# suilin0432/SoS-WSOD

Hardware: AMD Instinct MI355X
Metric: images/s (1/2/4/8 MI355X) VGG16+OICR 2000-prop; conv5_3 MFMA-util % (higher is better)
Workload: dtype bf16; 1 GPU; OICR+ training iteration: 4 views/step/GPU (1 image(s) x 2 scales x h-flip, every view 512x512), R=2000 proposals/view, K=20, VGG16 dilated-C5 + ROIPool 7x7 + fc6/fc7 4096 + WSDDN + 4 OICR heads, fwd+bwd+SGD(momentum, wd); image=one view, parallelism=dp1

## Files before the change

### include/soswsod_hip.h

```cpp
#ifndef SOSWSOD_HIP_H
#define SOSWSOD_HIP_H

#include <stdint.h>

#ifdef __cplusplus
extern "C" {
#endif

#ifndef SW_F32
#define SW_F32 0
#define SW_BF16 1
#endif

typedef struct ihipStream_t* sw_stream_t;

typedef struct sw_epilogue {
  const float* bias;
  int relu;
  const uint8_t* drop_mask;
  long ld_drop;
  float drop_scale;
  const void* relu_ref;
  long ld_ref;
  float ref_scale;
  int ref_dtype;
  int out_dtype;
  int accumulate_atomic;
  float* absmax_out;
  uint64_t drop_seed, drop_offset;
  float drop_hash_p;
  const uint64_t* drop_offset_dev;
  float* splitk_workspace;
  const void* residual;
  long ld_res;
  int res_dtype;
  const float* fold_row_scale;
  const struct sw_sgd_tensor_s* sgd_fused;
  float sgd_momentum, sgd_grad_scale;
} sw_epilogue;

int sw_gemm(int dtype, int a_kstrided, int b_kstrided, int M, int N, int K, const void* A, long lda, const void* B,
            long ldb, void* C, long ldc, const sw_epilogue* ep, int splitk, sw_stream_t stream);
long sw_gemm_splitk_workspace_floats(int M, int N, int K, int splitk);

int sw_conv3x3_igemm(int dtype, int nimg, int H, int W, int Cin, int Cout, int dilation, const void* in,
                     const void* wk, void* out, const sw_epilogue* ep, sw_stream_t stream);
int sw_conv3x3_relu_pool2(int dtype, int nimg, int H, int W, int Cin, int Cout, const void* in, const void* wk, const float* bias,
                          void* out_pooled, sw_stream_t stream);
typedef struct sw_conv_problem {
  int32_t nimg, H, W, Cin, Cout;
  const void* in; const void* wk; void* out;
  const sw_epilogue* ep;
} sw_conv_problem;
int sw_conv3x3_multi(int dtype, int n, const sw_conv_problem* probs, sw_stream_t stream);
long sw_conv3x3_wgrad_workspace_floats(int dtype, int nimg, int H, int W, int Cin, int Cout, int splitk);
int sw_conv3x3_wgrad(int dtype, int nimg, int H, int W, int Cin, int Cout, int dilation, const void* x, const void* dy,
                     float* dw_oihw, float* workspace, int splitk, const float* cout_scale, int accumulate, sw_stream_t stream);
int sw_conv3x3_wgrad_small(int dtype, int nimg, int H, int W, int Cin, int Cout, const void* x, const void* dy,
                           const float* cout_scale, float* dw_oihw, int accumulate, sw_stream_t stream);
int sw_conv3x3_wgrad_fold(int Cin, int Cout, int nslab, const float* workspace, float* dw_oihw, const float* cout_scale,
                          int accumulate, sw_stream_t stream);
typedef struct {
  int nimg, H, W, Cin, Cout, dilation, nsplit;
  const void* x;
  const void* dy;
  float* slabs;
} sw_wgrad_problem;
int sw_conv3x3_wgrad_grouped(int dtype, int n_problems, const sw_wgrad_problem* problems, sw_stream_t stream);
typedef struct sw_gemm_kk_problem {
  const void* A; const void* B; float* slabs;
  int32_t M, N, K, nsplit;
  long lda, ldb;
} sw_gemm_kk_problem;
int sw_gemm_kk_grouped(int dtype, int n_problems, const sw_gemm_kk_problem* problems, sw_stream_t stream);
long sw_gemm_kk_grouped_slabs(int dtype, int K, int nsplit);
typedef struct sw_splitk_fold { int32_t M, N, nslab, accumulate; const float* workspace; float* C; long ldc; const float* row_scale; } sw_splitk_fold;
int sw_splitk_fold_multi(int n, const sw_splitk_fold* folds, sw_stream_t stream);
typedef struct { int Cin, Cout, nslab; const float* workspace; float* dw_oihw; } sw_wgrad_fold;
int sw_conv3x3_wgrad_fold_multi(int n, const sw_wgrad_fold* folds, sw_stream_t stream);
int sw_conv_weight_prep(int dtype, int mode, int Cout, int Cin, int cin_pad, const float* w_oihw, void* wk,
                        sw_stream_t stream);

int sw_maxpool2x2_fwd(int dtype, int nimg, int H, int W, int C, int stride, const void* in, void* out,
                      sw_stream_t stream);
int sw_maxpool2x2_bwd(int dtype, int nimg, int H, int W, int C, int stride, const void* in, const void* dout,
                      void* din, int relu_mask, sw_stream_t stream);

int sw_preprocess(int dtype, int H, int W, int cpad, const uint8_t* img_chw, const float* mean3,
                  const float* std3, void* out_nhwc, sw_stream_t stream);
int sw_preprocess_multi(int dtype, int n, int H, int W, int cpad, const uint8_t* const* imgs_chw, const float* mean3,
                        const float* std3, void* out_nhwc, sw_stream_t stream);

long sw_roi_pool_fwd_workspace_bytes(int nimg, int R, int PH, int PW);
int sw_roi_pool_fwd(int dtype, int nimg, int H, int W, int C, int PH, int PW, float spatial_scale, const void* feat,
                    const float* rois, int R, const float* row_scale, float row_scale_add, void* out,
                    void* argmax, int argmax_bits, long ld_out, void* workspace, long workspace_bytes, sw_stream_t stream);
int sw_roi_pool_bwd(int dtype, int nimg, int H, int W, int C, int PH, int PW, const void* dout,
                    const void* argmax, int argmax_bits, long ld_in, const float* rois, int R, const float* row_scale,
                    float row_scale_add, const void* relu_ref, const float* dout_absmax, void* dfeat, float spatial_scale,
                    sw_stream_t stream);
int sw_absmax(int dtype, long n, const void* x, float* out, sw_stream_t stream);

long sw_wsddn_workspace_floats(int V, int R, int K);
int sw_wsddn_mil(int V, int R, int K, const float* logits, long ld, int cls_col, int det_col, const float* gt_onehot,
                 float* scores, float* loss_view, float* dlogits, long ld_d, const float* grad_scale,
                 float* mean_scores, long ld_mean, float* workspace, sw_stream_t stream);

long sw_wsddn_scores_bwd_workspace_floats(int R, int K);
int sw_wsddn_scores_bwd(int R, int K, const float* logits, long ld, const float* g_scores, long ld_g, float* dlogits, long ld_d,
                        float* workspace, sw_stream_t stream);
int sw_mean_views(int V, long n, const float* in, float* out, sw_stream_t stream);

int sw_oicr_mean_probs(int V, int R, int K, int n_rounds, const float* logits, long ld, int cls_col0, int col_stride,
                       float* out, sw_stream_t stream);

long sw_mine_workspace_bytes(int R, int top_k, int G);
int sw_oicr_mine_label(int R, int ncol, int K, int n_rounds, const float* scores, const int32_t* gt_classes, int G,
                       const float* boxes, int top_k, float score_thresh, float nms_thresh, float iou_bg,
                       float iou_fg, int32_t* lab_class, float* lab_weight, int32_t* lab_index, int32_t* pgt_count,
                       int32_t* pgt_index, int32_t* pgt_class, float* pgt_score, void* workspace,
                       sw_stream_t stream);

int sw_oicr_refine_loss(int V, int R, int K, int n_rounds, const float* logits, long ld, int cls_col, int box_col,
                        int col_stride, const float* boxes, const int32_t* lab_class, const float* lab_weight,
                        const int32_t* lab_index, const int32_t* pred_view, const float* reg_weights4,
                        float* loss_view, float* dlogits, long ld_d, const float* grad_scale, float* workspace,
                        sw_stream_t stream);

int sw_focal_loss(int N, int C, const float* logits, long ld, const int32_t* targets, float gamma, float* loss,
// ... 211 lines not shown
```

### sos-wsod_amd/_lib.py

```python
import ctypes
import os

import torch

_HERE = os.path.dirname(os.path.abspath(__file__))
LIB_PATH = os.environ.get("SW_LIB_PATH") or os.path.join(_HERE, "libsoswsod_hip.so")

SW_F32, SW_BF16 = 0, 1

c_int, c_long, c_float, c_void_p, c_u64 = ctypes.c_int, ctypes.c_long, ctypes.c_float, ctypes.c_void_p, ctypes.c_uint64
c_int32, c_uint32, c_double, c_longlong = ctypes.c_int32, ctypes.c_uint32, ctypes.c_double, ctypes.c_longlong


class Epilogue(ctypes.Structure):
    _fields_ = [
        ("bias", c_void_p), ("relu", c_int), ("drop_mask", c_void_p), ("ld_drop", c_long), ("drop_scale", c_float),
        ("relu_ref", c_void_p), ("ld_ref", c_long), ("ref_scale", c_float), ("ref_dtype", c_int),
        ("out_dtype", c_int), ("accumulate_atomic", c_int), ("absmax_out", c_void_p),
        ("drop_seed", c_u64), ("drop_offset", c_u64), ("drop_hash_p", c_float), ("drop_offset_dev", c_void_p),
        ("splitk_workspace", c_void_p),
        ("residual", c_void_p), ("ld_res", c_long), ("res_dtype", c_int),
        ("fold_row_scale", c_void_p),
        ("sgd_fused", c_void_p), ("sgd_momentum", c_float), ("sgd_grad_scale", c_float),
    ]


class WgradProblem(ctypes.Structure):
    _fields_ = [("nimg", c_int), ("H", c_int), ("W", c_int), ("Cin", c_int), ("Cout", c_int),
                ("dilation", c_int), ("nsplit", c_int), ("x", c_void_p), ("dy", c_void_p),
                ("slabs", c_void_p)]


class WgradFold(ctypes.Structure):
    _fields_ = [("Cin", c_int), ("Cout", c_int), ("nslab", c_int), ("workspace", c_void_p),
                ("dw_oihw", c_void_p)]


class AugRecipe(ctypes.Structure):
    _fields_ = [("seed", c_u64), ("key", c_u64), ("order", c_int32 * 4), ("factor", c_float * 4),
                ("hue_shift", c_int32), ("grayscale", c_int32), ("blur_r", c_int32),
                ("blur_ww", c_uint32), ("blur_fw", c_uint32), ("rect", (c_int32 * 4) * 3),
                ("pad_", c_int32)]


class AugItem(ctypes.Structure):
    _fields_ = [("src", c_void_p), ("out", c_void_p), ("tmp", c_void_p), ("lsum", c_void_p),
                ("H", c_int32), ("W", c_int32), ("recipe", AugRecipe)]


class GemmKKProblem(ctypes.Structure):
    _fields_ = [("A", c_void_p), ("B", c_void_p), ("slabs", c_void_p), ("M", c_int32), ("N", c_int32),
                ("K", c_int32), ("nsplit", c_int32), ("lda", c_long), ("ldb", c_long)]


class SplitkFold(ctypes.Structure):
    _fields_ = [("M", c_int32), ("N", c_int32), ("nslab", c_int32), ("accumulate", c_int32),
                ("workspace", c_void_p), ("C", c_void_p), ("ldc", c_long), ("row_scale", c_void_p)]


class ConvProblem(ctypes.Structure):
    _fields_ = [("nimg", c_int32), ("H", c_int32), ("W", c_int32), ("Cin", c_int32), ("Cout", c_int32),
                ("in_", c_void_p), ("wk", c_void_p), ("out", c_void_p), ("ep", ctypes.POINTER(Epilogue))]


class CopyDesc(ctypes.Structure):
    _fields_ = [("src", c_void_p), ("dst", c_void_p), ("bytes", c_long)]


class ColsumPart(ctypes.Structure):
    _fields_ = [("M", c_int), ("N", c_int), ("X", c_void_p), ("ld", c_long), ("workspace", c_void_p)]


class StageDesc(ctypes.Structure):
    _fields_ = [("w", c_void_p), ("bn_weight", c_void_p), ("bn_bias", c_void_p), ("bn_mean", c_void_p), ("bn_var", c_void_p),
                ("scale", c_void_p), ("shift", c_void_p), ("dst", c_void_p),
                ("kind", c_int32), ("rows", c_int32), ("cols", c_int32), ("block_start", c_int32)]


class ColsumFold(ctypes.Structure):
    _fields_ = [("N", c_int), ("n_partial_rows", c_int), ("workspace", c_void_p), ("out", c_void_p)]


class SgdTensor(ctypes.Structure):
    _fields_ = [
        ("param", c_void_p), ("grad", c_void_p), ("momentum_buf", c_void_p), ("n", c_long), ("lr", c_float),
        ("weight_decay", c_float), ("first_step", c_int), ("stage_kind", c_int), ("stage_dtype", c_int),
        ("stage0", c_void_p), ("stage1", c_void_p), ("d0", c_int), ("d1", c_int), ("d2", c_int), ("ld0", c_long), ("ld1", c_long),
        ("hyper_dev", c_void_p),
    ]


SGD_MAX_TENSORS = 24
_EP = ctypes.POINTER(Epilogue)
_F4 = ctypes.POINTER(c_float)

SIGNATURES = {
    "sw_gemm": (c_int, [c_int, c_int, c_int, c_int, c_int, c_int, c_void_p, c_long, c_void_p, c_long, c_void_p, c_long,
                        _EP, c_int, c_void_p]),
    "sw_gemm_splitk_workspace_floats": (c_long, [c_int, c_int, c_int, c_int]),
    "sw_gemm_sgd_fused_supported": (c_int, [c_int, c_int, c_int, c_int, c_int, c_int]),
    "sw_conv3x3_igemm": (c_int, [c_int, c_int, c_int, c_int, c_int, c_int, c_int, c_void_p, c_void_p, c_void_p, _EP,
                                 c_void_p]),
    "sw_conv3x3_wgrad": (c_int, [c_int, c_int, c_int, c_int, c_int, c_int, c_int, c_void_p, c_void_p, c_void_p, c_void_p,
                                 c_int, c_void_p, c_int, c_void_p]),
    "sw_conv3x3_wgrad_workspace_floats": (c_long, [c_int, c_int, c_int, c_int, c_int, c_int, c_int]),
    "sw_conv_weight_prep": (c_int, [c_int, c_int, c_int, c_int, c_int, c_void_p, c_void_p, c_void_p]),
    "sw_maxpool2x2_fwd": (c_int, [c_int, c_int, c_int, c_int, c_int, c_int, c_void_p, c_void_p, c_void_p]),
    "sw_maxpool2x2_bwd": (c_int, [c_int, c_int, c_int, c_int, c_int, c_int, c_void_p, c_void_p, c_void_p, c_int,
                                  c_void_p]),
    "sw_preprocess": (c_int, [c_int, c_int, c_int, c_int, c_void_p, _F4, _F4, c_void_p, c_void_p]),
    "sw_preprocess_multi": (c_int, [c_int, c_int, c_int, c_int, c_int, ctypes.POINTER(c_void_p), _F4, _F4, c_void_p, c_void_p]),
    "sw_roi_pool_fwd": (c_int, [c_int, c_int, c_int, c_int, c_int, c_int, c_int, c_float, c_void_p, c_void_p, c_int,
                                c_void_p, c_float, c_void_p, c_void_p, c_int, c_long, c_void_p, c_long, c_void_p]),
    "sw_roi_pool_fwd_workspace_bytes": (c_long, [c_int, c_int, c_int, c_int]),
    "sw_roi_pool_bwd": (c_int, [c_int, c_int, c_int, c_int, c_int, c_int, c_int, c_void_p, c_void_p, c_int, c_long, c_void_p, c_int,
                                c_void_p, c_float, c_void_p, c_void_p, c_void_p, c_float, c_void_p]),
    "sw_absmax": (c_int, [c_int, c_long, c_void_p, c_void_p, c_void_p]),
    "sw_wsddn_workspace_floats": (c_long, [c_int, c_int, c_int]),
    "sw_wsddn_mil": (c_int, [c_int, c_int, c_int, c_void_p, c_long, c_int, c_int, c_void_p, c_void_p, c_void_p,
                             c_void_p, c_long, c_void_p, c_void_p, c_long, c_void_p, c_void_p]),
    "sw_mean_views": (c_int, [c_int, c_long, c_void_p, c_void_p, c_void_p]),
    "sw_oicr_mean_probs": (c_int, [c_int, c_int, c_int, c_int, c_void_p, c_long, c_int, c_int, c_void_p, c_void_p]),
    "sw_mine_workspace_bytes": (c_long, [c_int, c_int, c_int]),
    "sw_oicr_mine_label": (c_int, [c_int, c_int, c_int, c_int, c_void_p, c_void_p, c_int, c_void_p, c_int, c_float, c_float,
                                   c_float, c_float, c_void_p, c_void_p, c_void_p, c_void_p, c_void_p, c_void_p,
                                   c_void_p, c_void_p, c_void_p]),
    "sw_oicr_refine_loss": (c_int, [c_int, c_int, c_int, c_int, c_void_p, c_long, c_int, c_int, c_int, c_void_p, c_void_p,
                                    c_void_p, c_void_p, c_void_p, _F4, c_void_p, c_void_p, c_long, c_void_p,
                                    c_void_p, c_void_p]),
    "sw_oicr_predict": (c_int, [c_int, c_int, c_int, c_void_p, c_long, c_int, c_int, c_void_p, _F4, c_float, c_void_p,
                                c_void_p, c_void_p]),
    "sw_detect_workspace_bytes": (c_long, [c_int, c_int, c_int]),
    "sw_detect_postprocess": (c_int, [c_int, c_int, c_void_p, c_void_p, c_int, c_int, c_float, c_float, c_int, c_void_p,
                                      c_void_p, c_void_p, c_void_p, c_void_p, c_void_p, c_long, c_void_p]),
    "sw_tta_merge": (c_int, [c_int, c_int, c_int, c_void_p, c_void_p, c_void_p, c_void_p, c_void_p, c_int, c_int, c_float, c_int,
                             c_void_p, c_void_p, c_void_p, c_void_p, c_void_p, c_void_p]),
    "sw_colsum": (c_int, [c_int, c_int, c_int, c_void_p, c_long, c_void_p, c_void_p, c_int, c_void_p]),
    "sw_colsum_workspace_floats": (c_long, [c_int, c_int, c_int]),
    "sw_conv3x3_wgrad_small": (c_int, [c_int, c_int, c_int, c_int, c_int, c_int, c_void_p, c_void_p, c_void_p, c_void_p, c_int, c_void_p]),
    "sw_conv3x3_wgrad_fold": (c_int, [c_int, c_int, c_int, c_void_p, c_void_p, c_void_p, c_int, c_void_p]),
    "sw_conv3x3_wgrad_fold_multi": (c_int, [c_int, ctypes.POINTER(WgradFold), c_void_p]),
    "sw_conv3x3_multi": (c_int, [c_int, c_int, ctypes.POINTER(ConvProblem), c_void_p]),
    "sw_gemm_kk_grouped": (c_int, [c_int, c_int, ctypes.POINTER(GemmKKProblem), c_void_p]),
    "sw_gemm_kk_grouped_slabs": (c_long, [c_int, c_int, c_int]),
    "sw_splitk_fold_multi": (c_int, [c_int, ctypes.POINTER(SplitkFold), c_void_p]),
    "sw_colsum_fold_multi": (c_int, [c_int, ctypes.POINTER(ColsumFold), c_void_p]),
    "sw_colsum_partial_multi": (c_int, [c_int, c_int, ctypes.POINTER(ColsumPart), c_void_p]),
    "sw_conv3x3_wgrad_grouped": (c_int, [c_int, c_int, ctypes.POINTER(WgradProblem), c_void_p]),
    "sw_convert_2d": (c_int, [c_int, c_int, c_int, c_void_p, c_long, c_void_p, c_long, c_void_p]),
    "sw_split_bf16x3": (c_int, [c_int, c_int, c_void_p, c_long, c_void_p, c_long, c_int, c_int, c_void_p]),
    "sw_nchw_to_nhwc": (c_int, [c_int, c_int, c_int, c_int, c_int, c_int, c_void_p, c_void_p, c_void_p]),
    "sw_relu_bwd": (c_int, [c_int, c_long, c_void_p, c_void_p, c_void_p, c_void_p]),
    "sw_scale_cols": (c_int, [c_int, c_int, c_int, c_void_p, c_long, c_void_p, c_void_p, c_long, c_void_p]),
    "sw_fill_zero": (c_int, [c_void_p, c_long, c_void_p]),
    "sw_dropout_mask": (c_int, [c_void_p, c_long, c_u64, c_u64, c_float, c_void_p]),
    "sw_sgd_momentum_step": (c_int, [c_void_p, c_void_p, c_void_p, c_long, c_float, c_float, c_float, c_int, c_float,
                                     c_void_p]),
    "sw_convert_2d_t": (c_int, [c_int, c_int, c_int, c_void_p, c_long, c_void_p, c_long, c_void_p]),
    "sw_sgd_multi": (c_int, [c_int, ctypes.POINTER(SgdTensor), c_float, c_float, c_void_p]),
    "sw_loss_finalize": (c_int, [c_int, c_int, c_int, c_void_p, c_void_p, c_void_p, c_void_p]),
    "sw_scale_cols_loss": (c_int, [c_int, c_int, c_int, c_int, c_void_p, c_long, c_void_p, c_void_p, c_void_p, c_float,
                                   c_void_p, c_long, c_void_p]),
    "sw_resize_pass_u8": (c_int, [c_int, c_int, c_int, c_long, c_long, c_int, c_int, c_void_p, c_void_p, c_void_p, c_int, c_void_p,
                                  c_void_p, c_void_p]),
    "sw_color_jitter_u8": (c_int, [c_int, c_int, c_int, c_void_p, c_float, c_double, c_float, c_void_p, c_void_p, c_void_p]),
    "sw_transpose_2d": (c_int, [c_int, c_int, c_int, c_void_p, c_long, c_void_p, c_long, c_void_p]),
    "sw_stage_blocks": (c_int, [c_int, c_int, c_int]),
    "sw_stage_weights_multi": (c_int, [c_int, c_int, c_void_p, c_int, c_float, c_void_p]),
    "sw_ema_multi": (c_int, [c_int, ctypes.POINTER(c_void_p), ctypes.POINTER(c_void_p), ctypes.POINTER(c_long), c_double, c_void_p]),
    "sw_threshold_select": (c_int, [c_int, c_void_p, c_void_p, c_void_p, c_float, c_void_p, c_int, c_void_p, c_void_p, c_void_p,
                                    c_void_p, c_void_p, c_void_p]),
    "sw_conv3x3_relu_pool2": (c_int, [c_int, c_int, c_int, c_int, c_int, c_int, c_void_p, c_void_p, c_void_p, c_void_p, c_void_p]),
    "sw_weighted_sum": (c_int, [c_int, c_void_p, c_void_p, c_void_p, c_void_p]),
    "sw_scale_scalars": (c_int, [c_int, c_void_p, c_void_p, c_void_p, c_void_p]),
    "sw_counter_add": (c_int, [c_void_p, c_u64, c_void_p]),
    "sw_focal_loss": (c_int, [c_int, c_int, c_void_p, c_long, c_void_p, c_float, c_void_p, c_void_p, c_long, c_void_p, c_void_p]),
    "sw_gaussian_blur_weights": (c_int, [c_float, ctypes.POINTER(c_int32), ctypes.POINTER(c_uint32),
                                         ctypes.POINTER(c_uint32)]),
    "sw_strong_aug_workspace_bytes": (c_long, [c_int, c_int]),
    "sw_strong_aug_u8": (c_int, [c_int, c_int, c_void_p, ctypes.POINTER(AugRecipe), c_void_p, c_void_p, c_void_p]),
    "sw_strong_aug_multi_u8": (c_int, [c_int, c_void_p, c_int, c_int, c_int, c_void_p]),
    "sw_copy_multi": (c_int, [c_int, ctypes.POINTER(CopyDesc), c_void_p]),
    "sw_pack_views": (c_int, [c_int, ctypes.POINTER(c_void_p), ctypes.POINTER(c_void_p), c_void_p, c_void_p, c_void_p,
                              c_void_p]),
    "sw_preprocess_pad": (c_int, [c_int, c_int, c_int, c_int, c_int, c_void_p, _F4, _F4, c_void_p, c_void_p]),
# ... 77 lines not shown
```

### sos-wsod_amd/backbone_vgg.py

```python
import os

import torch
import torch.nn as nn

from . import ops, staging
from .registry import BACKBONE_REGISTRY
from .structures import ShapeSpec

_STAGES = [("plain1", 3, 64, 2), ("plain2", 64, 128, 2), ("plain3", 128, 256, 3), ("plain4", 256, 512, 3),
           ("plain5", 512, 512, 3)]


def _epc(dtype):
    return 8 if dtype == torch.bfloat16 else 4


class _Conv(nn.Module):

    def __init__(self, cin, cout):
        super().__init__()
        self.weight = nn.Parameter(torch.empty(cout, cin, 3, 3))
        self.bias = nn.Parameter(torch.zeros(cout))
        nn.init.kaiming_normal_(self.weight, mode="fan_out", nonlinearity="relu")

# ... 134 lines not shown
                pi += 2
                cin = cur.shape[3]
                if (ci == blk.num_conv - 1 and blk.has_pool and blk.pool_stride == 2 and blk.dilation == 1 and dtype == torch.bfloat16
                        and (ft is None or bi < ft[0]) and cur.shape[1] >= 2 and cur.shape[2] >= 2):
                    oh, ow = (cur.shape[1] - 2) // 2 + 1, (cur.shape[2] - 2) // 2 + 1
                    pooled = torch.empty(cur.shape[0], oh, ow, blk.out_channels, device=x.device, dtype=dtype)
                    if ops.conv3x3_relu_pool2(cur, module.staged_weight(w, 0, cin, dtype), b, pooled, tag=f"{blk.tag}.conv{ci + 1}_fwd"):
                        conv_io.append((cur, None))
                        cur = pooled
                        continue
                out = torch.empty(cur.shape[0], cur.shape[1], cur.shape[2], blk.out_channels, device=x.device, dtype=dtype)
                ep = ops.make_epilogue(bias=b, relu=True, out_dtype=dtype)
                if module.x3_layer(dtype, cin, blk.out_channels):
                    n_, h_, w_ = cur.shape[:3]
                    x3 = ops.split_bf16x3(cur.view(n_ * h_ * w_, cin), 0,
                                          out=torch.empty(n_ * h_ * w_, 6 * cin, device=x.device, dtype=torch.bfloat16))
                    ops.conv3x3(x3.view(n_, h_, w_, 6 * cin), module.staged_weight_x3(w, 0, cin), out, blk.dilation, ep,
                                tag=f"{blk.tag}.conv{ci + 1}_fwd")
                else:
                    wk = module.staged_weight(w, 0, cin, dtype)
                    ops.conv3x3(cur, wk, out, blk.dilation, ep, tag=f"{blk.tag}.conv{ci + 1}_fwd")
                conv_io.append((cur, out))
                cur = out
            pre_pool = None
            if blk.has_pool and conv_io[-1][1] is not None:
                pre_pool = cur
                s = blk.pool_stride
                oh, ow = (cur.shape[1] - 2) // s + 1, (cur.shape[2] - 2) // s + 1
                pooled = torch.empty(cur.shape[0], oh, ow, cur.shape[3], device=x.device, dtype=dtype)
                ops.maxpool_fwd(cur, pooled, s)
                cur = pooled
            stage_info.append((conv_io, pre_pool))
        return cur, stage_info

    @staticmethod
    def backward(ctx, *gs):
        module, infos, params = ctx.module, ctx.infos, ctx.params
        ctx.infos = None
        n_in = len(infos)
        grads = [None] * len(params)
        first_trainable = module.first_trainable_conv()
        live = [i for i in range(n_in) if gs[i] is not None]
        if first_trainable is None or not live:
            return (None, None) + (None,) * n_in + tuple(grads)
        dev = gs[live[0]].device
        dtype = infos[0][0][0][0][0].dtype
        main = torch.cuda.current_stream()
        side = module.side_stream() if len(live) > 1 else None
        x3w = False
        if module.fp32x3 and dtype == torch.float32:
            x3w, pj = True, len(params)
            for sj in range(len(module.blocks) - 1, -1, -1):
                for cj in range(module.blocks[sj].num_conv - 1, -1, -1):
                    pj -= 2
                    if params[pj].requires_grad and not module.x3_layer(dtype, infos[live[0]][sj][0][cj][0].shape[3], module.blocks[sj].out_channels):
                        x3w = False
        wdt, nmul = (torch.bfloat16, 6) if x3w else (dtype, 1)
        bk = 64 if wdt == torch.bfloat16 else 32
        deferred = []
        module._colsum_deferred = []
        shapes, probs6, keys = [], [], []
        pj = len(params)
        for sj in range(len(module.blocks) - 1, -1, -1):
            bj = module.blocks[sj]
            for cj in range(bj.num_conv - 1, -1, -1):
                pj -= 2
                if params[pj].requires_grad:
                    for i in live:
                        xin = infos[i][sj][0][cj][0]
                        shapes.append((nmul * xin.shape[0] * xin.shape[1] * xin.shape[2], bj.out_channels, 9 * xin.shape[3]))
                        probs6.append((nmul * xin.shape[0], xin.shape[1], xin.shape[2], xin.shape[3], bj.out_channels, bj.dilation))
                        keys.append((pj, i))
        direct_ns = dict(zip(keys, _wgrad_direct_splits(probs6))) if _wgrad_direct_covers(probs6, wdt) else None
        target = _wgrad_grouped_target(shapes, bk)
        plan = {}
        pidx = len(params)
        for si in range(len(module.blocks) - 1, -1, -1):
            blk = module.blocks[si]
            for ci in range(blk.num_conv - 1, -1, -1):
                pidx -= 2
                w = params[pidx]
                if w.requires_grad:
                    cout = blk.out_channels
                    slab_off, row_off, nslab, nrow, splits = {}, {}, 0, 0, {}
                    for i in live:
                        x_in = infos[i][si][0][ci][0]
                        n, H, W, cin = x_in.shape
                        splits[i] = (direct_ns[(pidx, i)] if direct_ns is not None
                                     else _wgrad_grouped_splits(nmul * n * H * W, bk, target))
                        slab_off[i], row_off[i] = nslab, nrow
                        nslab += ops.conv3x3_wgrad_nslab_shape(wdt, nmul * n, H, W, cin, cout, splits[i])
                        nrow += ops.colsum_nrows(dtype, n * H * W, cout)
                    cin = infos[live[0]][si][0][ci][0].shape[3]
                    plan[pidx] = dict(ws=torch.empty(nslab, cout * 9 * cin, device=dev, dtype=torch.float32),
                                      rows=torch.empty(nrow, cout, device=dev, dtype=torch.float32), slab_off=slab_off,
                                      row_off=row_off, nslab=nslab, nrow=nrow, splits=splits, cin=cin,
                                      dw=ops.grad_target(w, (cout, cin, 3, 3), dev),
                                      db=ops.grad_target(params[pidx + 1], (cout,), dev))
                if (si, ci) == first_trainable:
                    break
            if si == first_trainable[0]:
                break
        if side is not None:
            side.wait_stream(main)
        for k, i in enumerate(live):
            st = side if (side is not None and k % 2 == 1) else main
            with torch.cuda.stream(st):
                g = gs[i]
                if st is not main:
                    g.record_stream(st)
                _VGGFunction._backward_one(module, infos[i], params, g, dtype, plan, i, first_trainable,
                                           deferred, None if st is main else main, x3w)
            infos[i] = None
        if side is not None:
            main.wait_stream(side)
        if deferred:
            ops.conv3x3_wgrad_grouped(deferred, tag="wgrad_grouped")
            ops.colsum_partial_multi(module._colsum_deferred)
            deferred.clear()
        module._colsum_deferred = []
        ops.conv3x3_wgrad_fold_multi([(pl["ws"], pl["nslab"], pl["dw"]) for pl in plan.values()])
        ops.colsum_fold_multi([(pl["rows"], pl["nrow"], pl["db"]) for pl in plan.values()])
        for pidx, pl in plan.items():
            w = params[pidx]
            grads[pidx] = pl["dw"][:, : w.shape[1]].contiguous() if pl["cin"] != w.shape[1] else pl["dw"]
            grads[pidx + 1] = pl["db"]
        return (None, None) + (None,) * n_in + tuple(grads)

    @staticmethod
    def _backward_one(module, stage_info, params, g, dtype, plan, i, first_trainable, deferred, consumer_stream, x3w=False):
        g = g.contiguous()
        if g.dtype != dtype:
            g = g.to(dtype)
        last_out = stage_info[-1][0][-1][1]
        assert stage_info[-1][1] is None, "backward expects the last stage to have no pool (vgg.py:197)"
        dz = ops.relu_bwd(last_out, g, out=torch.empty_like(g))
        pidx = len(params)
        for si in range(len(stage_info) - 1, -1, -1):
            blk = module.blocks[si]
            conv_io, _ = stage_info[si]
            for ci in range(blk.num_conv - 1, -1, -1):
                pidx -= 2
                x_in, _ = conv_io[ci]
                w = params[pidx]
                n, H, W, cin = x_in.shape
                pl = plan.get(pidx)
                if pl is not None:
                    npix = n * H * W
                    xw, dw_ = x_in, dz
                    if x3w:
                        cout = blk.out_channels
                        xw = ops.split_bf16x3(x_in.view(npix, cin), 1, along_rows=True,
                                              out=torch.empty(6 * npix, cin, device=g.device, dtype=torch.bfloat16)).view(6 * n, H, W, cin)
                        dw_ = ops.split_bf16x3(dz.view(npix, cout), 0, along_rows=True,
                                               out=torch.empty(6 * npix, cout, device=g.device, dtype=torch.bfloat16)).view(6 * n, H, W, cout)
                    if consumer_stream is not None:
                        xw.record_stream(consumer_stream); dw_.record_stream(consumer_stream)
                        dz.record_stream(consumer_stream)
                    deferred.append((xw, dw_, pl["ws"][pl["slab_off"][i]:], blk.dilation, pl["splits"][i]))
                    module._colsum_deferred.append((dz.view(npix, blk.out_channels), pl["rows"][pl["row_off"][i]:]))
                if (si, ci) == first_trainable:
                    return
                dx = torch.empty(n, H, W, cin, device=g.device, dtype=dtype)
                ref = x_in.view(n * H * W, cin) if ci > 0 else None
                epd = ops.make_epilogue(relu_ref=ref, out_dtype=dtype)
                if module.x3_layer(dtype, blk.out_channels, cin):
                    cout = blk.out_channels
                    dz3 = ops.split_bf16x3(dz.view(n * H * W, cout), 0,
                                           out=torch.empty(n * H * W, 6 * cout, device=g.device, dtype=torch.bfloat16))
                    ops.conv3x3(dz3.view(n, H, W, 6 * cout), module.staged_weight_x3(w, 1, cin), dx, blk.dilation, epd,
                                tag=f"{blk.tag}.conv{ci + 1}_dgrad")
                else:
                    wkd = module.staged_weight(w, 1, cin, dtype)
                    ops.conv3x3(dz, wkd, dx, blk.dilation, epd, tag=f"{blk.tag}.conv{ci + 1}_dgrad")
                dz = dx
            prev_pre_pool = stage_info[si - 1][1]
            pblk = module.blocks[si - 1]
            din = torch.empty_like(prev_pre_pool)
            ops.maxpool_bwd(prev_pre_pool, dz, din, pblk.pool_stride, relu_mask=True)
            dz = din


class VGG16(nn.Module):

    def __init__(self, conv5_dilation, freeze_at, num_classes=None, out_features=None, compute_dtype=torch.bfloat16):
        super().__init__()
        self.num_classes = num_classes
        self.compute_dtype = compute_dtype
        self.dual_stream = True
        self._side = None
        self._stage = staging.StageCache()
        self._stage_x3 = staging.StageCache()
        self.fp32x3 = (compute_dtype == torch.float32 and os.environ.get("SW_FP32X3", "0") == "1"
                       and os.environ.get("SW_FP32X3_CONV", "1") != "0")
        self._out_feature_strides, self._out_feature_channels = {}, {}
        self.stages_and_names = []
        strides = {"plain1": 2, "plain2": 4, "plain3": 8, "plain4": 8 if conv5_dilation == 2 else 16,
                   "plain5": 8 if conv5_dilation == 2 else 16}
        self.blocks = []
        for i, (name, cin, cout, nconv) in enumerate(_STAGES):
            if name == "plain4":
                blk = PlainBlock(cin, cout, num_conv=nconv, stride=1 if conv5_dilation == 2 else 2, has_pool=True)
            elif name == "plain5":
                blk = PlainBlock(cin, cout, num_conv=nconv, stride=1, dilation=conv5_dilation, has_pool=False)
            else:
                blk = PlainBlock(cin, cout, num_conv=nconv, stride=2, has_pool=True)
            stage = nn.Sequential(blk)
            self.add_module(name, stage)
            self.stages_and_names.append((stage, name))
            blk.tag = name
            self.blocks.append(blk)
            self._out_feature_strides[name] = strides[name]
            self._out_feature_channels[name] = cout
            if freeze_at >= i + 1:
                blk.freeze()
        if out_features is None:
            out_features = ["plain5"]
        self._out_features = out_features
        assert self._out_features == ["plain5"], "this build exposes the hot path's feature only (IN_FEATURES ['plain5'])"

    @property
    def size_divisibility(self):
        return 0

    def staged_weight(self, w, mode, cin_pad, dtype):
        cout, cin = w.shape[:2]
        shape = (cout, 9, cin_pad) if mode == 0 else (cin, 9, cout)
        slot, built = self._stage.lookup((id(w), mode), (w,), (shape,), dtype, w.device, alloc=torch.zeros,
                                         build=lambda b: ops.conv_weight_prep(w.detach(), b[0], mode, cin_pad if mode == 0 else None))
        if built and w.requires_grad:
            both = [self._stage.get((id(w), m)) for m in (0, 1)]
            both = [s if s is not None and s.bufs[0].dtype == dtype else None for s in both]
            b0, b1 = (None if s is None else s.bufs[0] for s in both)
            staging.register(w, 2, dtype, stage0=b0, stage1=b1, d0=cout, d1=cin, d2=cin if b0 is None else b0.shape[2],
                             slots=[(s, 0) for s in both if s is not None])
        return slot.bufs[0]

    def x3_layer(self, dtype, cin, cout):
        return self.fp32x3 and dtype == torch.float32 and cin % 64 == 0 and cout % 64 == 0

    def staged_weight_x3(self, w, mode, cin_pad):
        n, k = (w.shape[0], cin_pad) if mode == 0 else (w.shape[1], w.shape[0])
        return self._stage_x3.lookup((id(w), mode), (w,), ((n, 9, 6 * k),), torch.bfloat16, w.device, lambda b: ops.split_bf16x3(
            self.staged_weight(w, mode, cin_pad, torch.float32).view(9 * n, k), 1, out=b[0].view(9 * n, 6 * k)))[0].bufs[0]

    def stage_all_weights(self, with_dgrad):
        dtype = self.compute_dtype
        epc = _epc(dtype)
# ... 67 lines not shown
```

### sos-wsod_amd/csrc/conv_direct.hip

```cpp
#include <type_traits>
#include "common.h"
#include "soswsod_hip.h"

namespace {

constexpr int TH = 8, TW = 32, CK = 32;
constexpr unsigned INVALID = 0xFFFFFF00u;

struct DirectArgs {
  const void* in; const void* wk; void* out;
  const float* bias; const void* ref;
  int nimg, H, W, Cin, Cout, relu;
  int pool;
  int out_f32;
  int tiles_x, tiles_y, n_px_tiles, n_co_blocks, total;
  unsigned in_bytes, wk_bytes;
};

template <int N> __device__ __forceinline__ void wait_vm() { asm volatile("s_waitcnt vmcnt(%0)" ::"n"(N) : "memory"); }

template <int DIL, int TN, int KG = 1>
__device__ __forceinline__ void conv3x3_direct_body(const DirectArgs& g, const unsigned bid) {
  static_assert(KG == 1 || (KG == 2 && TN == 64), "K groups: two groups of four waves, 64-channel tiles");
  constexpr int DEPTH = 2;
  constexpr int NI = TN / 16;
  constexpr int B_INSTR = 3 * TN * 4 / 64, B_PER_WAVE = (B_INSTR + 3) / 4;
  constexpr int PH = TH + 2 * DIL, PW = TW + 2 * DIL, P = PH * PW;
  constexpr int A_INSTR = (P * 4 + 63) / 64;
  constexpr int A_PER_WAVE = (A_INSTR + 3) / 4;
  constexpr int A_BYTES = A_PER_WAVE * 4 * 1024;
  constexpr int B_BYTES = 3 * TN * 64;
  typedef __attribute__((address_space(3))) void* lvoid;
  extern __shared__ __attribute__((aligned(16))) char smem[];
  const int tid = threadIdx.x, lane = tid & 63;
  const int wave_all = __builtin_amdgcn_readfirstlane(tid >> 6);
  const int grp = KG == 1 ? 0 : (wave_all >> 2), wave = wave_all & 3;
  char* const sA = smem + grp * (2 * A_BYTES);
  char* const sB = smem + KG * 2 * A_BYTES + grp * (DEPTH * B_BYTES);

  const int per_xcd = (g.total + 7) >> 3;
  const int f = (bid & 7) * per_xcd + (bid >> 3);
  if ((int)(bid >> 3) >= per_xcd || f >= g.total) return;
  const int px_tile = f / g.n_co_blocks, co_blk = f - px_tile * g.n_co_blocks;
  const int img = px_tile / (g.tiles_x * g.tiles_y);
  const int trem = px_tile - img * (g.tiles_x * g.tiles_y);
  const int ty0 = (trem / g.tiles_x) * TH, tx0 = (trem % g.tiles_x) * TW;
  const int co0 = co_blk * TN;

  const __amdgpu_buffer_rsrc_t rsA = __builtin_amdgcn_make_buffer_rsrc((void*)g.in, 0, (int)g.in_bytes, 0x00020000);
  const __amdgpu_buffer_rsrc_t rsB = __builtin_amdgcn_make_buffer_rsrc((void*)g.wk, 0, (int)g.wk_bytes, 0x00020000);

  unsigned a_v[A_PER_WAVE];
#pragma unroll
  for (int s = 0; s < A_PER_WAVE; ++s) {
    const int q = wave + 4 * s;
    const int idx = q * 64 + lane;
    const int prow = idx >> 2, p = idx & 3;
    const int src = p ^ (((prow >> 2) & 1) << 1);
    const int py = prow / PW, px = prow - py * PW;
    const int y = ty0 - DIL + py, x = tx0 - DIL + px;
    const bool ok = prow < P && y >= 0 && y < g.H && x >= 0 && x < g.W;
    a_v[s] = ok ? (unsigned)(((((long)img * g.H + y) * g.W + x) * g.Cin + src * 8) * 2) : INVALID;
  }
  unsigned b_v[B_PER_WAVE];
#pragma unroll
  for (int s = 0; s < B_PER_WAVE; ++s) {
    const int idx = (wave + 4 * s) * 64 + lane;
    const int r = idx >> 2, p = idx & 3;
    const int tap_x = r / TN, co = r - tap_x * TN;
    const int src = p ^ (((co >> 2) & 1) << 1);
    const bool ok = tap_x < 3 && co0 + co < g.Cout;
    b_v[s] = ok ? (unsigned)((((long)(co0 + co) * 9 + tap_x) * g.Cin + src * 8) * 2) : INVALID;
  }
  auto issue_a = [&](int chunk) {
    char* dst = sA + (chunk & 1) * A_BYTES;
    const unsigned soff = (unsigned)(chunk * KG + grp) * (CK * 2);
#pragma unroll
    for (int s = 0; s < A_PER_WAVE; ++s)
      __builtin_amdgcn_raw_ptr_buffer_load_lds(rsA, (lvoid)(dst + (wave + 4 * s) * 1024), 16, (int)a_v[s], (int)soff, 0, 0);
  };
  auto issue_b = [&](int step) {
    const int chunk = step / 3, ty = step - chunk * 3;
    char* dst = sB + (step % DEPTH) * B_BYTES;
    const unsigned soff = (unsigned)((ty * 3 * g.Cin + (chunk * KG + grp) * CK) * 2);
#pragma unroll
    for (int s = 0; s < B_PER_WAVE; ++s)
      if (wave + 4 * s < B_INSTR)
        __builtin_amdgcn_raw_ptr_buffer_load_lds(rsB, (lvoid)(dst + (wave + 4 * s) * 1024), 16, (int)b_v[s], (int)soff, 0, 0);
  };

  f32x4 acc[4][NI];
#pragma unroll
  for (int i = 0; i < 4; ++i)
#pragma unroll
    for (int j = 0; j < NI; ++j) acc[i][j] = f32x4{0.f, 0.f, 0.f, 0.f};

  const int nchunk = g.Cin / (CK * KG), nstep = nchunk * 3;
  const int l15 = lane & 15, kq = lane >> 4;
  int b_off[NI];
#pragma unroll
// ... 48 lines not shown
        if (step + 1 < nstep) issue_b(step + 1);
        if (ty == 0 && chunk + 1 < nchunk) issue_a(chunk + 1);
        if (FORM != FORM_EMPTY) compute_step(par_c, ty_c);
      };
      one(std::integral_constant<int, 0>{}); one(std::integral_constant<int, 1>{}); one(std::integral_constant<int, 2>{});
    };
    for (int chunk = 0; chunk < nchunk; chunk += 2) {
      chunk_steps(std::integral_constant<int, 0>{}, chunk);
      if (chunk + 1 < nchunk) chunk_steps(std::integral_constant<int, 1>{}, chunk + 1);
    }
  };
  {
    static_assert(TW == 32 && TH == 8, "edge forms: 16-pixel sub-tiles, two rows per wave");
    const bool left_only = tx0 + 16 >= g.W;
    const bool no_rows = ty0 + 2 * wave >= g.H;
    if (no_rows) main_loop(std::integral_constant<int, FORM_EMPTY>{});
    else if (left_only) main_loop(std::integral_constant<int, FORM_LEFT>{});
    else main_loop(std::integral_constant<int, FORM_FULL>{});
  }
  __syncthreads();

  unsigned short* out = (unsigned short*)g.out;
  const unsigned short* ref = (const unsigned short*)g.ref;
  if (KG == 2) {
    f32x4* X = (f32x4*)smem;
#pragma unroll
    for (int i2 = 0; i2 < 2; ++i2)
#pragma unroll
      for (int j = 0; j < NI; ++j) {
        const f32x4 give = grp == 0 ? acc[2 + i2][j] : acc[i2][j];
        X[((wave_all * 2 + i2) * NI + j) * 64 + lane] = give;
      }
    __syncthreads();
    f32x4 fin[2][NI];
#pragma unroll
    for (int i2 = 0; i2 < 2; ++i2)
#pragma unroll
      for (int j = 0; j < NI; ++j) {
        const f32x4 got = X[(((wave_all ^ 4) * 2 + i2) * NI + j) * 64 + lane];
        const f32x4 mine = grp == 0 ? acc[i2][j] : acc[2 + i2][j];
        fin[i2][j] = grp == 0 ? f32x4{mine[0] + got[0], mine[1] + got[1], mine[2] + got[2], mine[3] + got[3]}
                              : f32x4{got[0] + mine[0], got[1] + mine[1], got[2] + mine[2], got[3] + mine[3]};
      }
    if (g.out_f32) {
      float* outf = (float*)g.out;
      const float* reff = (const float*)g.ref;
      const int y = ty0 + 2 * wave + grp;
#pragma unroll
      for (int j = 0; j < NI; ++j) {
        const int co = co0 + j * 16 + l15;
        const float bv = (g.bias && co < g.Cout) ? g.bias[co] : 0.f;
#pragma unroll
        for (int i2 = 0; i2 < 2; ++i2)
#pragma unroll
          for (int e = 0; e < 4; ++e) {
            const int x = tx0 + i2 * 16 + kq * 4 + e;
            if (y < g.H && x < g.W && co < g.Cout) {
              float v = fin[i2][j][e] + bv;
              if (g.relu) v = relu_keep_nan(v);
              const long o = (((long)img * g.H + y) * g.W + x) * g.Cout + co;
              if (reff && !(reff[o] > 0.f)) v = 0.f;
              outf[o] = v;
            }
          }
      }
      return;
    }
    unsigned short* S = (unsigned short*)(smem + 8 * 2 * NI * 64 * 16 + wave_all * (32 * TN * 2));
#pragma unroll
    for (int j = 0; j < NI; ++j) {
      const int col = j * 16 + l15;
      const float bv = (g.bias && co0 + col < g.Cout) ? g.bias[co0 + col] : 0.f;
#pragma unroll
      for (int i2 = 0; i2 < 2; ++i2)
#pragma unroll
        for (int e = 0; e < 4; ++e) {
          float v = fin[i2][j][e] + bv;
          if (g.relu) v = relu_keep_nan(v);
          const int pl = i2 * 16 + kq * 4 + e;
          S[pl * TN + (col ^ ((pl & (TN / 8 - 1)) << 3))] = f32_to_bf16_bits(v);
        }
    }
    __builtin_amdgcn_s_waitcnt(0xc07f);
#pragma unroll
    for (int it = 0; it < TN / 16; ++it) {
      const int idx = it * 64 + lane;
      const int pl = idx / (TN / 8), ch = idx % (TN / 8);
      const int y = ty0 + 2 * wave + grp, x = tx0 + pl;
      const int co = co0 + ch * 8;
      if (y < g.H && x < g.W && co < g.Cout) {
        u32x4 v = *(const u32x4*)(S + pl * TN + ((ch ^ (pl & (TN / 8 - 1))) << 3));
        const long o = (((long)img * g.H + y) * g.W + x) * g.Cout + co;
        if (ref) {
          const u32x4 r = *(const u32x4*)(ref + o);
#pragma unroll
          for (int t = 0; t < 4; ++t) {
            const bool lo = __uint_as_float(r[t] << 16) > 0.f, hi = __uint_as_float(r[t] & 0xFFFF0000u) > 0.f;
            v[t] = (lo ? (v[t] & 0xFFFFu) : 0u) | (hi ? (v[t] & 0xFFFF0000u) : 0u);
          }
        }
        *(u32x4*)(out + o) = v;
      }
    }
    return;
  }
  if (g.out_f32) {
    float* outf = (float*)g.out;
    const float* reff = (const float*)g.ref;
#pragma unroll
    for (int j = 0; j < NI; ++j) {
      const int co = co0 + j * 16 + l15;
      const float bv = (g.bias && co < g.Cout) ? g.bias[co] : 0.f;
#pragma unroll
      for (int i = 0; i < 4; ++i)
#pragma unroll
        for (int e = 0; e < 4; ++e) {
          const int pl = i * 16 + kq * 4 + e;
          const int y = ty0 + 2 * wave + (pl >> 5), x = tx0 + (pl & 31);
          if (y < g.H && x < g.W && co < g.Cout) {
            float v = acc[i][j][e] + bv;
            if (g.relu) v = relu_keep_nan(v);
            const long o = (((long)img * g.H + y) * g.W + x) * g.Cout + co;
            if (reff && !(reff[o] > 0.f)) v = 0.f;
            outf[o] = v;
          }
        }
    }
    return;
  }
  unsigned short* S = (unsigned short*)(smem + wave * (64 * TN * 2));
#pragma unroll
  for (int j = 0; j < NI; ++j) {
    const int col = j * 16 + l15;
    const float bv = (g.bias && co0 + col < g.Cout) ? g.bias[co0 + col] : 0.f;
#pragma unroll
    for (int i = 0; i < 4; ++i)
#pragma unroll
      for (int e = 0; e < 4; ++e) {
        float v = acc[i][j][e] + bv;
        if (g.relu) v = relu_keep_nan(v);
        const int pl = i * 16 + kq * 4 + e;
        S[pl * TN + (col ^ ((pl & (TN / 8 - 1)) << 3))] = f32_to_bf16_bits(v);
      }
  }
  __builtin_amdgcn_s_waitcnt(0xc07f);
  if (g.pool) {
    const int OH = (g.H - 2) / 2 + 1, OW = (g.W - 2) / 2 + 1;
#pragma unroll
    for (int it = 0; it < (16 * (TN / 8) + 63) / 64; ++it) {
      const int idx = it * 64 + lane;
      const int pp = idx / (TN / 8), ch = idx % (TN / 8);
      const int oy = (ty0 + 2 * wave) >> 1, ox = (tx0 >> 1) + pp;
      const int co = co0 + ch * 8;
      if (pp < 16 && oy < OH && ox < OW && co < g.Cout) {
        float a[8];
#pragma unroll
        for (int t = 0; t < 4; ++t) {
          const int pl = (t >> 1) * 32 + 2 * pp + (t & 1);
          const u32x4 v = *(const u32x4*)(S + pl * TN + ((ch ^ (pl & (TN / 8 - 1))) << 3));
#pragma unroll
          for (int q = 0; q < 4; ++q) {
            const float lo = __uint_as_float(v[q] << 16), hi = __uint_as_float(v[q] & 0xFFFF0000u);
            a[2 * q] = t == 0 ? lo : max_keep_nan(a[2 * q], lo);
            a[2 * q + 1] = t == 0 ? hi : max_keep_nan(a[2 * q + 1], hi);
          }
        }
        u32x4 o;
#pragma unroll
        for (int q = 0; q < 4; ++q) o[q] = (unsigned)f32_to_bf16_bits(a[2 * q]) | ((unsigned)f32_to_bf16_bits(a[2 * q + 1]) << 16);
        *(u32x4*)(out + (((long)img * OH + oy) * OW + ox) * g.Cout + co) = o;
      }
    }
    return;
  }
#pragma unroll
  for (int it = 0; it < TN / 8; ++it) {
    const int idx = it * 64 + lane;
    const int pl = idx / (TN / 8), ch = idx % (TN / 8);
    const int y = ty0 + 2 * wave + (pl >> 5), x = tx0 + (pl & 31);
    const int co = co0 + ch * 8;
    if (y < g.H && x < g.W && co < g.Cout) {
      u32x4 v = *(const u32x4*)(S + pl * TN + ((ch ^ (pl & (TN / 8 - 1))) << 3));
      const long o = (((long)img * g.H + y) * g.W + x) * g.Cout + co;
      if (ref) {
        const u32x4 r = *(const u32x4*)(ref + o);
#pragma unroll
        for (int t = 0; t < 4; ++t) {
          const bool lo = __uint_as_float(r[t] << 16) > 0.f, hi = __uint_as_float(r[t] & 0xFFFF0000u) > 0.f;
          v[t] = (lo ? (v[t] & 0xFFFFu) : 0u) | (hi ? (v[t] & 0xFFFF0000u) : 0u);
        }
      }
      *(u32x4*)(out + o) = v;
    }
  }
}

template <int DIL, int TN, int KG = 1>
__global__ __launch_bounds__(256 * KG, KG == 1 ? 2 : 1) void conv3x3_direct_kernel(DirectArgs g) {
  conv3x3_direct_body<DIL, TN, KG>(g, blockIdx.x);
}

constexpr int DIRECT_MULTI_MAX = 8;
struct DirectMulti {
  int n;
  unsigned first[DIRECT_MULTI_MAX + 1];
  DirectArgs p[DIRECT_MULTI_MAX];
};
__global__ __launch_bounds__(256, 2) void conv3x3_direct_multi_kernel(DirectMulti m) {
  int i = 0;
  while (i + 1 < m.n && blockIdx.x >= m.first[i + 1]) ++i;
  conv3x3_direct_body<1, 64, 1>(m.p[i], blockIdx.x - m.first[i]);
}

__global__ __launch_bounds__(256) void conv3x3_first_kernel(int nimg, int H, int W, const unsigned short* __restrict__ in,
                                                            const unsigned short* __restrict__ wk,
                                                            const float* __restrict__ bias, int relu,
                                                            unsigned short* __restrict__ out) {
  __shared__ __attribute__((aligned(16))) unsigned short S_all[4][64 * 64];
  const int lane = threadIdx.x & 63, wave = threadIdx.x >> 6;
  const int l15 = lane & 15, kq = lane >> 4;
  unsigned short* S = S_all[wave];
  u32x4 fb[4][3];
#pragma unroll
  for (int j = 0; j < 4; ++j)
#pragma unroll
    for (int s3 = 0; s3 < 3; ++s3) {
      const int tap = s3 * 4 + kq;
      fb[j][s3] = tap < 9 ? *(const u32x4*)(wk + ((long)(j * 16 + l15) * 9 + tap) * 8) : u32x4{0u, 0u, 0u, 0u};
    }
  float bv[4];
#pragma unroll
  for (int j = 0; j < 4; ++j) bv[j] = bias ? bias[j * 16 + l15] : 0.f;
  int dy[3], dx[3];
#pragma unroll
  for (int s3 = 0; s3 < 3; ++s3) { const int tap = s3 * 4 + kq; dy[s3] = tap / 3 - 1; dx[s3] = tap % 3 - 1; }
  const int segs = (W + 63) / 64;
  const long nseg = (long)nimg * H * segs;
  for (long sg = (long)blockIdx.x * 4 + wave; sg < nseg; sg += (long)gridDim.x * 4) {
    const int xs = (int)(sg % segs) * 64; const long t = sg / segs;
    const int y = (int)(t % H), img = (int)(t / H);
    f32x4 acc[4][4];
#pragma unroll
    for (int i = 0; i < 4; ++i)
#pragma unroll
      for (int j = 0; j < 4; ++j) acc[i][j] = f32x4{0.f, 0.f, 0.f, 0.f};
#pragma unroll
    for (int i = 0; i < 4; ++i) {
      const int x = xs + i * 16 + l15;
      u32x4 fa[3];
#pragma unroll
      for (int s3 = 0; s3 < 3; ++s3) {
        const int yy = y + dy[s3], xx = x + dx[s3];
        const bool ok = s3 * 4 + kq < 9 && yy >= 0 && yy < H && xx >= 0 && xx < W;
        fa[s3] = ok ? *(const u32x4*)(in + (((long)img * H + yy) * W + xx) * 8) : u32x4{0u, 0u, 0u, 0u};
      }
#pragma unroll
      for (int s3 = 0; s3 < 3; ++s3)
#pragma unroll
        for (int j = 0; j < 4; ++j)
          acc[i][j] = __builtin_amdgcn_mfma_f32_16x16x32_bf16(__builtin_bit_cast(bf16x8, fa[s3]), __builtin_bit_cast(bf16x8, fb[j][s3]),
                                                              acc[i][j], 0, 0, 0);
    }
#pragma unroll
    for (int j = 0; j < 4; ++j)
#pragma unroll
      for (int i = 0; i < 4; ++i)
#pragma unroll
        for (int e = 0; e < 4; ++e) {
          float v = acc[i][j][e] + bv[j];
          if (relu) v = relu_keep_nan(v);
          const int pl = i * 16 + kq * 4 + e, col = j * 16 + l15;
          S[pl * 64 + (col ^ ((pl & 7) << 3))] = f32_to_bf16_bits(v);
        }
#pragma unroll
    for (int it = 0; it < 8; ++it) {
      const int idx = it * 64 + lane;
      const int pl = idx >> 3, ch = idx & 7;
      const int x = xs + pl;
      if (x < W)
        *(u32x4*)(out + (((long)img * H + y) * W + x) * 64 + ch * 8) = *(const u32x4*)(S + pl * 64 + ((ch ^ (pl & 7)) << 3));
    }
  }
}

}

int sw_conv3x3_direct_try(int nimg, int H, int W, int Cin, int Cout, int dilation, const void* in, const void* wk, void* out,
                          const sw_epilogue* ep, hipStream_t stream) {
  if (Cin == 8 && Cout == 64 && dilation == 1 && ep && ep->out_dtype == SW_BF16 && !ep->drop_mask && !ep->relu_ref &&
      !ep->accumulate_atomic && !ep->absmax_out && !(ep->drop_hash_p > 0.f) &&
      (((uintptr_t)in | (uintptr_t)wk | (uintptr_t)out) & 15) == 0) {
    const long nseg = (long)nimg * H * ((W + 63) / 64);
    long blocks = (nseg + 3) / 4;
    if (blocks > 4096) blocks = 4096;
    hipLaunchKernelGGL(conv3x3_first_kernel, dim3((unsigned)blocks), dim3(256), 0, stream, nimg, H, W, (const unsigned short*)in,
                       (const unsigned short*)wk, ep->bias, ep->relu, (unsigned short*)out);
    hipError_t e1 = hipGetLastError();
    return e1 == hipSuccess ? 1 : -(int)e1;
  }
  if ((Cin % CK) || (Cout % 8) || (dilation != 1 && dilation != 2)) return 0;
  if (ep && ((ep->out_dtype != SW_BF16 && ep->out_dtype != SW_F32) || ep->drop_mask || ep->accumulate_atomic || ep->absmax_out)) return 0;
  if (!ep) return 0;
  if (ep->relu_ref && (ep->ref_dtype != ep->out_dtype || ep->ld_ref != Cout || ep->ref_scale != 1.0f)) return 0;
  if (ep->residual || ep->drop_hash_p > 0.f) return 0;
  if ((((uintptr_t)in | (uintptr_t)wk | (uintptr_t)out | (uintptr_t)ep->relu_ref) & 15)) return 0;
  if (Cin < 64) return 0;
  DirectArgs g = {};
  g.in = in; g.wk = wk; g.out = out; g.bias = ep->bias; g.ref = ep->relu_ref; g.relu = ep->relu;
  g.out_f32 = ep->out_dtype == SW_F32;
  g.nimg = nimg; g.H = H; g.W = W; g.Cin = Cin; g.Cout = Cout;
  g.tiles_x = (W + TW - 1) / TW; g.tiles_y = (H + TH - 1) / TH;
  g.n_px_tiles = g.tiles_x * g.tiles_y * nimg;
  const bool few = g.n_px_tiles * ((Cout + 63) / 64) <= 384;
  const int kg = (few && (Cin % (2 * CK)) == 0) ? 2 : 1;
  const int tn = (few && kg == 1) ? 32 : 64;
  g.n_co_blocks = (Cout + tn - 1) / tn;
  g.total = g.n_px_tiles * g.n_co_blocks;
  const long ib = (long)nimg * H * W * Cin * 2, wb = (long)Cout * 9 * Cin * 2;
  if (ib >= 0xFFFFFF00L || wb >= 0xFFFFFF00L) return 0;
  g.in_bytes = (unsigned)ib; g.wk_bytes = (unsigned)wb;
  const int per_xcd = (g.total + 7) / 8;
  const int d = dilation;
  const int P = (TH + 2 * d) * (TW + 2 * d);
  const int apw = ((P * 4 + 63) / 64 + 3) / 4;
  const size_t lds = (size_t)kg * ((size_t)2 * apw * 4096 + (size_t)2 * (3 * tn * 64));
  hipError_t e = hipSuccess;
#define SW_LAUNCH_DIRECT(D, TNV, KGV)                                                                                     \
  do {                                                                                                                     \
    auto kern = conv3x3_direct_kernel<D, TNV, KGV>;                                                                        \
    e = hipFuncSetAttribute((const void*)kern, hipFuncAttributeMaxDynamicSharedMemorySize, (int)lds);                      \
    if (e != hipSuccess) return -(int)e;                                                                                   \
    hipLaunchKernelGGL(kern, dim3(per_xcd * 8), dim3(256 * kg), lds, stream, g);                                           \
  } while (0)
  if (kg == 2) { if (d == 1) SW_LAUNCH_DIRECT(1, 64, 2); else SW_LAUNCH_DIRECT(2, 64, 2); }
  else if (tn == 32) { if (d == 1) SW_LAUNCH_DIRECT(1, 32, 1); else SW_LAUNCH_DIRECT(2, 32, 1); }
  else { if (d == 1) SW_LAUNCH_DIRECT(1, 64, 1); else SW_LAUNCH_DIRECT(2, 64, 1); }
#undef SW_LAUNCH_DIRECT
  e = hipGetLastError();
  if (e != hipSuccess) return -(int)e;
  return 1;
}


extern "C" int sw_conv3x3_relu_pool2(int dtype, int nimg, int H, int W, int Cin, int Cout, const void* in, const void* wk, const float* bias,
                                     void* out_pooled, hipStream_t stream) {
  SW_ENTER();
  if (dtype != SW_BF16 || (Cin % CK) || Cin < 64 || (Cout % 64) || H < 2 || W < 2) return 0;
  if ((((uintptr_t)in | (uintptr_t)wk | (uintptr_t)out_pooled) & 15)) return 0;
  DirectArgs g = {};
  g.in = in; g.wk = wk; g.out = out_pooled; g.bias = bias; g.ref = nullptr; g.relu = 1; g.pool = 1;
  g.nimg = nimg; g.H = H; g.W = W; g.Cin = Cin; g.Cout = Cout;
  g.tiles_x = (W + TW - 1) / TW; g.tiles_y = (H + TH - 1) / TH;
  g.n_px_tiles = g.tiles_x * g.tiles_y * nimg;
  g.n_co_blocks = Cout / 64;
  g.total = g.n_px_tiles * g.n_co_blocks;
  if (g.total <= 384) return 0;
  const long ib = (long)nimg * H * W * Cin * 2, wb = (long)Cout * 9 * Cin * 2;
  if (ib >= 0xFFFFFF00L || wb >= 0xFFFFFF00L) return 0;
  g.in_bytes = (unsigned)ib; g.wk_bytes = (unsigned)wb;
  const int per_xcd = (g.total + 7) / 8;
  constexpr int P = (TH + 2) * (TW + 2);
  constexpr int apw = ((P * 4 + 63) / 64 + 3) / 4;
  const size_t lds = (size_t)2 * apw * 4096 + (size_t)2 * (3 * 64 * 64);
  auto kern = conv3x3_direct_kernel<1, 64, 1>;
  hipError_t e = hipFuncSetAttribute((const void*)kern, hipFuncAttributeMaxDynamicSharedMemorySize, (int)lds);
  if (e != hipSuccess) return -(int)e;
  hipLaunchKernelGGL(kern, dim3(per_xcd * 8), dim3(256), lds, stream, g);
  e = hipGetLastError();
  return e == hipSuccess ? 1 : -(int)e;
}


extern "C" int sw_conv3x3_multi(int dtype, int n, const sw_conv_problem* probs, hipStream_t stream) {
  SW_ENTER();
  if (n <= 0) return 1;
  if (dtype != SW_BF16 || n > DIRECT_MULTI_MAX) return 0;
  DirectMulti m = {};
  m.n = n;
  unsigned wgs = 0;
  for (int i = 0; i < n; ++i) {
    const sw_conv_problem& q = probs[i];
    const sw_epilogue* ep = q.ep;
    if (!ep || q.nimg <= 0 || q.H <= 0 || q.W <= 0) return 0;
    if ((q.Cin % CK) || q.Cin < 64 || (q.Cout % 8)) return 0;
    if (ep->out_dtype != SW_BF16 || ep->drop_mask || ep->accumulate_atomic || ep->absmax_out || (ep->drop_hash_p > 0.f) || ep->residual) return 0;
    if (ep->relu_ref && (ep->ref_dtype != SW_BF16 || ep->ld_ref != q.Cout || ep->ref_scale != 1.0f)) return 0;
    if ((((uintptr_t)q.in | (uintptr_t)q.wk | (uintptr_t)q.out | (uintptr_t)ep->relu_ref) & 15)) return 0;
    DirectArgs& g = m.p[i];
    g.in = q.in; g.wk = q.wk; g.out = q.out; g.bias = ep->bias; g.ref = ep->relu_ref; g.relu = ep->relu;
    g.nimg = q.nimg; g.H = q.H; g.W = q.W; g.Cin = q.Cin; g.Cout = q.Cout;
    g.tiles_x = (q.W + TW - 1) / TW; g.tiles_y = (q.H + TH - 1) / TH;
    g.n_px_tiles = g.tiles_x * g.tiles_y * q.nimg;
    g.n_co_blocks = (q.Cout + 63) / 64;
    g.total = g.n_px_tiles * g.n_co_blocks;
    const long ib = (long)q.nimg * q.H * q.W * q.Cin * 2, wb = (long)q.Cout * 9 * q.Cin * 2;
    if (ib >= 0xFFFFFF00L || wb >= 0xFFFFFF00L) return 0;
    g.in_bytes = (unsigned)ib; g.wk_bytes = (unsigned)wb;
    m.first[i] = wgs;
    wgs += (unsigned)(((g.total + 7) / 8) * 8);
  }
  m.first[n] = wgs;
  constexpr int P = (TH + 2) * (TW + 2);
  constexpr int apw = ((P * 4 + 63) / 64 + 3) / 4;
  constexpr size_t lds = (size_t)2 * apw * 4096 + (size_t)2 * (3 * 64 * 64);
  hipError_t e = hipFuncSetAttribute((const void*)conv3x3_direct_multi_kernel, hipFuncAttributeMaxDynamicSharedMemorySize, (int)lds);
  if (e != hipSuccess) return -(int)e;
  hipLaunchKernelGGL(conv3x3_direct_multi_kernel, dim3(wgs), dim3(256), lds, stream, m);
  e = hipGetLastError();
  if (e != hipSuccess) return -(int)e;
  return 1;
}
```

### sos-wsod_amd/csrc/gemm.hip

```cpp
#include "common.h"
#include "soswsod_hip.h"

namespace {

enum { OP_KCONTIG = 0, OP_KSTRIDED = 1, OP_CONV_A = 2, OP_CONV_B = 3, OP_CONV_A_GEN = 4 };

struct GemmArgs {
  const void* A; const void* B; void* C;
  int M, N, K;
  long lda, ldb, ldc;
  int tiles_m, tiles_n, patches_m, k_per_split;
  int patch_m_log2;
  int cH, cW, cC, cDil;
  const float* bias;
  const uint8_t* drop; long ldd; float drop_scale;
  unsigned long long drop_seed_mixed, drop_offset; float drop_p;
  const unsigned long long* drop_offset_dev;
  const void* ref; long ldr; float ref_scale; int ref_bf16;
  const void* res; long ldres; int res_bf16;
  int relu, out_bf16, atomic, oihw_cin, staged_out;
  unsigned a_bytes, b_bytes;
  long slab_stride;
  int vgrid;
  int krot;
  float* absmax;
  float* sgd_param; float* sgd_mom; long sgd_ld;
  unsigned short* sgd_st0; long sgd_ld0; unsigned short* sgd_st1; long sgd_ld1;
  const float* sgd_hyper; float sgd_lr, sgd_wd, sgd_momentum, sgd_gscale; int sgd_first;
};

template <typename T> struct GT;
template <> struct GT<unsigned short> { static constexpr int EPC = 8, BK = 64; };
template <> struct GT<float> { static constexpr int EPC = 4, BK = 32; };

__device__ const u32x4 g_zero_chunk = {0u, 0u, 0u, 0u};


template <typename T> struct Mma;
template <> struct Mma<unsigned short> {
  static constexpr int TS = 16, NSTEP = 2, NACC = 4;
  typedef f32x4 Acc;
  __device__ static __forceinline__ void mma(Acc& acc, const u32x4& a, const u32x4& b) {
    acc = __builtin_amdgcn_mfma_f32_16x16x32_bf16(__builtin_bit_cast(bf16x8, a), __builtin_bit_cast(bf16x8, b), acc, 0, 0, 0);
  }
  __device__ static __forceinline__ int row(int lane, int e) { return (lane >> 4) * 4 + e; }
  __device__ static __forceinline__ int col(int lane) { return lane & 15; }
};
template <> struct Mma<float> {
  static constexpr int TS = 32, NSTEP = 4, NACC = 16;
  typedef f32x16 Acc;
  __device__ static __forceinline__ void mma(Acc& acc, const u32x4& a, const u32x4& b) {
#pragma unroll
    for (int t = 0; t < 4; ++t)
      acc = __builtin_amdgcn_mfma_f32_32x32x2f32(__uint_as_float(a[t]), __uint_as_float(b[t]), acc, 0, 0, 0);
  }
  __device__ static __forceinline__ int row(int lane, int e) { return (e & 3) + 8 * (e >> 2) + 4 * (lane >> 5); }
  __device__ static __forceinline__ int col(int lane) { return lane & 31; }
};

template <typename T, int MODE, int ROWS_MN>
struct Geom2 {
  static constexpr bool KS = (MODE == OP_KSTRIDED || MODE == OP_CONV_B);
  static constexpr int BK = GT<T>::BK;
  static constexpr int CPR = KS ? (ROWS_MN * (int)sizeof(T) / 16) : 8;
  static constexpr int NROW = KS ? BK : ROWS_MN;
  static constexpr int BYTES = NROW * CPR * 16;
  static constexpr int ROW_BYTES = CPR * 16;
  __device__ static __forceinline__ int swz(int row) {
    if (!KS) return (row >> 1) & 7;
    if (sizeof(T) == 2) return ((row & 3) << 2) | (Mma<T>::TS == 16 ? ((row >> 3) & 1) << 1 : 0);
    return 0;
  }
};

template <typename T, bool KS, int ROW_BYTES>
__device__ __forceinline__ u32x4 load_frag2(const char* tile, int sub_base, int s, int lane) {
  constexpr int TS = Mma<T>::TS;
  if (!KS) {
    const int row = sub_base + (lane & (TS - 1));
    const int chunk = TS == 32 ? 2 * s + (lane >> 5) : 4 * s + (lane >> 4);
    return *(const u32x4*)(tile + row * 128 + ((chunk ^ ((row >> 1) & 7)) << 4));
  } else if (sizeof(T) == 2) {
    const int G = lane >> 4, i16 = lane & 15, q = i16 >> 2, p = i16 & 3;
    const int col = TS == 32 ? sub_base + 16 * (G & 1) + 4 * p : sub_base + 4 * p;
    const int chunk = col >> 3, half = (col >> 2) & 1;
    const int row0 = TS == 32 ? 16 * s + 8 * (G >> 1) + q : 32 * s + 8 * G + q;
    const int row1 = row0 + 4;
    const int off0 = row0 * ROW_BYTES + ((chunk ^ Geom2<T, OP_KSTRIDED, 128>::swz(row0)) << 4) + half * 8;
    const int off1 = row1 * ROW_BYTES + ((chunk ^ Geom2<T, OP_KSTRIDED, 128>::swz(row1)) << 4) + half * 8;
    typedef __attribute__((address_space(3))) s16x4 lds_s16x4;
    s16x4 lo = __builtin_amdgcn_ds_read_tr16_b64_v4i16((lds_s16x4*)(tile + off0));
    s16x4 hi = __builtin_amdgcn_ds_read_tr16_b64_v4i16((lds_s16x4*)(tile + off1));
    u32x2 l2 = __builtin_bit_cast(u32x2, lo), h2 = __builtin_bit_cast(u32x2, hi);
    u32x4 o; o[0] = l2[0]; o[1] = l2[1]; o[2] = h2[0]; o[3] = h2[1];
    return o;
  } else {
    const int r = lane & 31, h = lane >> 5;
    const int col = sub_base + r;
    u32x4 o;
#pragma unroll
    for (int t = 0; t < 4; ++t) o[t] = *(const unsigned int*)(tile + (8 * s + 4 * h + t) * ROW_BYTES + col * 4);
    return o;
  }
}

template <int V> struct IntC { static constexpr int value = V; };

template <int N> __device__ __forceinline__ void wait_vmcnt() {
  static_assert(N >= 0 && N < 64, "vmcnt is a 6-bit field");
  asm volatile("s_waitcnt vmcnt(%0)" ::"n"(N) : "memory");
}
// ... 250 lines not shown
    };
    if (nt > 0) { issue_begin(0); issue_range(0, GROUP); }
    dma_pair(1, 0);
    tile_wait(-1);
    __builtin_amdgcn_s_barrier();
    if (grp == 1) __builtin_amdgcn_s_barrier();
    u32x4 fa[QI][NSTEP], fb[2][QJ][NSTEP];
    for (int kt = 0; kt < nt; ++kt) {
      const char* sa = smem + (kt & 1) * STAGE_BYTES;
      const char* sb = sa + GA::BYTES;
      auto phase = [&](auto pc) {
        constexpr int p = decltype(pc)::value;
        constexpr int mq = p >> 1, nq = (p == 1 || p == 2) ? 1 : 0;
        __builtin_amdgcn_sched_barrier(0);
        if (p == 0 || p == 2) {
#pragma unroll
          for (int ii = 0; ii < QI; ++ii)
#pragma unroll
            for (int st = 0; st < NSTEP; ++st) fa[ii][st] = load_frag2<T, GA::KS, GA::ROW_BYTES>(sa, wm * WTM + (mq * QI + ii) * TS, st, lane);
        }
        if (p == 0 || p == 1) {
#pragma unroll
          for (int jj = 0; jj < QJ; ++jj)
#pragma unroll
            for (int st = 0; st < NSTEP; ++st) fb[nq][jj][st] = load_frag2<T, GB::KS, GB::ROW_BYTES>(sb, wn * WTN + (nq * QJ + jj) * TS, st, lane);
        }
        if (p == 3) dma_pair(kt + 2, 0); else dma_pair(kt + 1, p + 1);
        if (grp == 1 && p == 2) asm volatile("s_waitcnt lgkmcnt(0)" ::: "memory");
        if (grp == 1 && p == 3) tile_wait(kt);
        __builtin_amdgcn_sched_barrier(0);
        __builtin_amdgcn_s_barrier();
        __builtin_amdgcn_sched_barrier(0);
        asm volatile("s_waitcnt lgkmcnt(0)" ::: "memory");
        __builtin_amdgcn_s_setprio(1);
#pragma unroll
        for (int st = 0; st < NSTEP; ++st)
#pragma unroll
          for (int ii = 0; ii < QI; ++ii)
#pragma unroll
            for (int jj = 0; jj < QJ; ++jj) MM::mma(acc[mq * QI + ii][nq * QJ + jj], fa[ii][st], fb[nq][jj][st]);
        __builtin_amdgcn_s_setprio(0);
        if (grp == 0 && p == 3) tile_wait(kt);
        __builtin_amdgcn_sched_barrier(0);
        __builtin_amdgcn_s_barrier();
        __builtin_amdgcn_sched_barrier(0);
      };
      phase(IntC<0>{}); phase(IntC<1>{}); phase(IntC<2>{}); phase(IntC<3>{});
    }
    if (grp == 0) __builtin_amdgcn_s_barrier();
  } else {
#pragma unroll
  for (int t = 0; t < STAGES - 1; ++t)
    if (t < nt) stage_issue(t);

  for (int kt = 0; kt < nt; ++kt) {
    if (kt + STAGES - 2 < nt) wait_vmcnt<GROUP * (STAGES - 2)>();
    else wait_vmcnt<0>();
    __builtin_amdgcn_s_barrier();
    const bool refill = kt + STAGES - 1 < nt;
    if (STAGES >= 3) {
      if (refill) issue_begin(kt + STAGES - 1);
      compute(kt, refill);
      if (refill) issue_end();
    } else {
      if (refill) stage_issue(kt + STAGES - 1);
      compute(kt, false);
    }
  }
  }

  const int r = MM::col(lane);
  unsigned int vmax = 0u;
  const unsigned long long drop_base = g.drop_seed_mixed + g.drop_offset + ((g.drop_p > 0.f && g.drop_offset_dev) ? *g.drop_offset_dev : 0ull);
  if constexpr (PP) {
    constexpr int LDW = WTN + 4;
    float* wt = (float*)smem + wave * (32 * LDW);
    constexpr int TP = 40;
    unsigned short* tT = (unsigned short*)((float*)smem + NW * (32 * LDW)) + wave * (WTN * TP);
    static_assert((long)NW * (32 * LDW) * 4 + (long)NW * WTN * TP * 2 <= (long)STAGES * STAGE_BYTES, "epilogue staging fits the ring");
    float sgd_lr = g.sgd_lr, sgd_wd = g.sgd_wd;
    if (g.sgd_param && g.sgd_hyper) { sgd_lr = g.sgd_hyper[0]; sgd_wd = g.sgd_hyper[1]; }
    __syncthreads();
    const bool vec_ok = g.staged_out;
    auto quarter = [&](auto qc) {
      constexpr int q = decltype(qc)::value;
      constexpr int NPC = (32 * (WTN / 4)) / 64;
      f32x4 pw[NPC], pm[NPC];
      if (g.sgd_param) {
        const int nbq = n0t + wn * WTN + (lane % (WTN / 4)) * 4;
#pragma unroll
        for (int it = 0; it < NPC; ++it) {
          const int mq = m0 + wm * WTM + q * 32 + (it * 64 + lane) / (WTN / 4);
          const bool okq = mq < g.M && nbq < g.N;
          const long po = (long)mq * g.sgd_ld + nbq;
          pw[it] = okq ? *(const f32x4*)(g.sgd_param + po) : f32x4{0.f, 0.f, 0.f, 0.f};
          pm[it] = (okq && !g.sgd_first) ? *(const f32x4*)(g.sgd_mom + po) : f32x4{0.f, 0.f, 0.f, 0.f};
        }
      }
#pragma unroll
      for (int ii = 0; ii < 32 / TS; ++ii)
#pragma unroll
        for (int j = 0; j < NI; ++j)
#pragma unroll
          for (int e = 0; e < NACC; ++e) wt[(ii * TS + MM::row(lane, e)) * LDW + j * TS + r] = acc[(32 / TS) * q + ii][j][e];
      __builtin_amdgcn_s_waitcnt(0xc07f);
      auto pieces = [&](auto cpc, auto plainc) {
        constexpr int CP = decltype(cpc)::value;
        constexpr bool PLAIN = decltype(plainc)::value != 0;
        constexpr int PPR = WTN / CP;
        const int c0 = (lane % PPR) * CP;
        const int nb = n0t + wn * WTN + c0;
        float bcol[CP];
#pragma unroll
        for (int t = 0; t < CP; ++t) bcol[t] = (!PLAIN && g.bias && nb + t < g.N) ? g.bias[nb + t] : 0.f;
        const bool ref_vec = !PLAIN && g.ref && g.ref_bf16 && CP == 8 && (g.ldr % 8) == 0 && ((((uintptr_t)g.ref) & 15) == 0);
#pragma unroll
        for (int it = 0; it < (32 * PPR) / 64; ++it) {
          const int pc = it * 64 + lane;
          const int row = pc / PPR;
          const int m = m0 + wm * WTM + q * 32 + row;
          if (m >= g.M || nb >= g.N) continue;
          float v[CP];
          *(f32x4*)&v[0] = *(const f32x4*)&wt[row * LDW + c0];
          if (CP == 8) *(f32x4*)&v[CP - 4] = *(const f32x4*)&wt[row * LDW + c0 + 4];
          const bool full = nb + CP <= g.N;
          u32x4 refw = {0u, 0u, 0u, 0u};
          const bool ref_piece = ref_vec && full;
          if (ref_piece) refw = *(const u32x4*)((const unsigned short*)g.ref + (long)m * g.ldr + nb);
#pragma unroll
          for (int t = 0; t < CP; ++t) {
            const int n = nb + t;
            const bool ok = n < g.N;
            float x = v[t];
            if (!PLAIN) {
              x += bcol[t];
              if (g.res && ok) x += g.res_bf16 ? bf16_bits_to_f32(((const unsigned short*)g.res)[(long)m * g.ldres + n])
                                               : ((const float*)g.res)[(long)m * g.ldres + n];
              if (g.relu) x = relu_keep_nan(x);
              if (g.drop && ok) x = g.drop[(long)m * g.ldd + n] ? x * g.drop_scale : 0.f;
              if (g.drop_p > 0.f && ok) {
                unsigned long long z = drop_base + (unsigned long long)((long)m * g.N + n);
                z += 0x9E3779B97F4A7C15ull;
                z = (z ^ (z >> 30)) * 0xBF58476D1CE4E5B9ull;
                z = (z ^ (z >> 27)) * 0x94D049BB133111EBull;
                z ^= z >> 31;
                const float u = (float)(z >> 40) * (1.0f / 16777216.0f);
                x = u >= g.drop_p ? x * g.drop_scale : 0.f;
              }
              if (g.ref && ok) {
                float rv;
                if (ref_piece) rv = __uint_as_float((t & 1) ? (refw[(t >> 1) & 3] & 0xFFFF0000u) : (refw[(t >> 1) & 3] << 16));
                else rv = g.ref_bf16 ? bf16_bits_to_f32(((const unsigned short*)g.ref)[(long)m * g.ldr + n])
                                     : ((const float*)g.ref)[(long)m * g.ldr + n];
                x = rv > 0.f ? x * g.ref_scale : 0.f;
              }
            }
            if (ok) vmax = max(vmax, absbits(x));
            v[t] = x;
          }
          const long o = (long)m * g.ldc + nb;
          if (CP == 4 && PLAIN && g.sgd_param) {
            const long po = (long)m * g.sgd_ld + nb;
            const f32x4 w4 = pw[it * CP / 4 < NPC ? it * CP / 4 : 0];
            f32x4 m4 = pm[it * CP / 4 < NPC ? it * CP / 4 : 0];
            f32x4 wn;
#pragma unroll
            for (int t = 0; t < 4; ++t) {
              const float dd = v[t] * g.sgd_gscale + sgd_wd * w4[t];
              m4[t] = g.sgd_first ? dd : g.sgd_momentum * m4[t] + dd;
              wn[t] = w4[t] - sgd_lr * m4[t];
            }
            *(f32x4*)(g.sgd_mom + po) = m4;
            *(f32x4*)(g.sgd_param + po) = wn;
            const unsigned b01 = (unsigned)f32_to_bf16_bits(wn[0]) | ((unsigned)f32_to_bf16_bits(wn[1]) << 16);
            const unsigned b23 = (unsigned)f32_to_bf16_bits(wn[2]) | ((unsigned)f32_to_bf16_bits(wn[3]) << 16);
            if (g.sgd_st0) *(u32x2*)(g.sgd_st0 + (long)m * g.sgd_ld0 + nb) = u32x2{b01, b23};
            if (g.sgd_st1) {
              tT[(c0 + 0) * TP + row] = (unsigned short)(b01 & 0xFFFFu); tT[(c0 + 1) * TP + row] = (unsigned short)(b01 >> 16);
              tT[(c0 + 2) * TP + row] = (unsigned short)(b23 & 0xFFFFu); tT[(c0 + 3) * TP + row] = (unsigned short)(b23 >> 16);
            }
            continue;
          }
          if (CP == 4) {
            if (g.atomic && g.slab_stride <= 0) {
#pragma unroll
              for (int t = 0; t < 4; ++t) if (nb + t < g.N) atomicAdd((float*)g.C + o + t, v[t]);
            } else {
              float* dst = (float*)g.C + o + (g.slab_stride > 0 ? (long)zsplit * g.slab_stride : 0);
              if (full && vec_ok) __builtin_nontemporal_store(*(const f32x4*)&v[0], (f32x4*)dst);
              else {
#pragma unroll
                for (int t = 0; t < 4; ++t) if (nb + t < g.N) dst[t] = v[t];
              }
            }
          } else {
            unsigned short* dst = (unsigned short*)g.C + o;
            if (full && vec_ok) {
              u32x4 w;
#pragma unroll
              for (int t = 0; t < 4; ++t) w[t] = (unsigned)f32_to_bf16_bits(v[2 * t]) | ((unsigned)f32_to_bf16_bits(v[2 * t + 1]) << 16);
              __builtin_nontemporal_store(w, (u32x4*)dst);
            } else {
#pragma unroll
              for (int t = 0; t < CP; ++t) if (nb + t < g.N) dst[t] = f32_to_bf16_bits(v[t]);
            }
          }
        }
      };
      const bool plain_ep = !g.bias && !g.relu && !g.drop && !(g.drop_p > 0.f) && !g.ref && !g.res;
      const bool bf16_rows = g.out_bf16 && g.slab_stride <= 0 && !g.atomic;
      if (bf16_rows) { if (plain_ep) pieces(IntC<8>{}, IntC<1>{}); else pieces(IntC<8>{}, IntC<0>{}); }
      else { if (plain_ep) pieces(IntC<4>{}, IntC<1>{}); else pieces(IntC<4>{}, IntC<0>{}); }
      if (g.sgd_param && g.sgd_st1) {
        __builtin_amdgcn_s_waitcnt(0xc07f);
        const int part = lane & 3;
        const int mrow = m0 + wm * WTM + q * 32 + part * 8;
#pragma unroll
        for (int ps = 0; ps < WTN / 16; ++ps) {
          const int c = ps * 16 + (lane >> 2);
          const int n = n0t + wn * WTN + c;
          if (n < g.N && mrow < g.M)
            *(u32x4*)(g.sgd_st1 + (long)n * g.sgd_ld1 + mrow) = *(const u32x4*)(tT + c * TP + part * 8);
        }
      }
    };
    quarter(IntC<0>{}); quarter(IntC<1>{}); quarter(IntC<2>{}); quarter(IntC<3>{});
  } else {
  const bool staged = g.staged_out;
  unsigned short* stile = (unsigned short*)smem + wave * (WTM * WTN);
  if (staged) __syncthreads();
  const bool res_staged = staged && g.res && g.res_bf16 && (g.ldres % 8) == 0 && ((((uintptr_t)g.res) & 15) == 0);
  const bool ref_ok = staged && g.ref && g.ref_bf16 && (g.ldr % 8) == 0 && ((((uintptr_t)g.ref) & 15) == 0);
  const bool ref_staged = ref_ok && !g.res;
  constexpr bool TWO_TILES = 2L * NW * WTM * WTN * 2 <= (long)STAGES * STAGE_BYTES;
  const bool ref_staged2 = TWO_TILES && ref_ok && res_staged;
  unsigned short* stile2 = stile + NW * (WTM * WTN);
  auto fetch_tile = [&](const unsigned short* src, const long lds_, unsigned short* dst) {
    constexpr int CPRW = WTN / 8;
#pragma unroll
    for (int q = 0; q < (WTM * CPRW) / 64; ++q) {
      const int idx = q * 64 + lane, lrow = idx / CPRW, ch = idx % CPRW;
      const int m = m0 + wm * WTM + lrow, n = n0t + wn * WTN + ch * 8;
      u32x4 rv = {0u, 0u, 0u, 0u};
      if (m < g.M && n < g.N) rv = *(const u32x4*)(src + (long)m * lds_ + n);
      *(u32x4*)(dst + lrow * WTN + ch * 8) = rv;
    }
  };
  if (res_staged || ref_staged) {
    if (res_staged) fetch_tile((const unsigned short*)g.res, g.ldres, stile);
    else fetch_tile((const unsigned short*)g.ref, g.ldr, stile);
    if (ref_staged2) fetch_tile((const unsigned short*)g.ref, g.ldr, stile2);
    __builtin_amdgcn_fence(__ATOMIC_ACQ_REL, "wavefront");
    __builtin_amdgcn_wave_barrier();
  }
#pragma unroll
  for (int i = 0; i < MI; ++i)
#pragma unroll
    for (int j = 0; j < NI; ++j) {
      const int n = n0t + wn * WTN + j * TS + r;
      const bool nok = n < g.N;
      const float bcol = (g.bias && nok) ? g.bias[n] : 0.f;
#pragma unroll
      for (int e = 0; e < NACC; ++e) {
        const int lrow = i * TS + MM::row(lane, e);
        const int m = m0 + wm * WTM + lrow;
        const bool ok = nok && m < g.M;
        float v = acc[i][j][e] + bcol;
        if (res_staged) v += bf16_bits_to_f32(stile[lrow * WTN + j * TS + r]);
        else if (g.res && ok) v += g.res_bf16 ? bf16_bits_to_f32(((const unsigned short*)g.res)[(long)m * g.ldres + n])
                                              : ((const float*)g.res)[(long)m * g.ldres + n];
        if (g.relu) v = relu_keep_nan(v);
        if (g.drop && ok) v = g.drop[(long)m * g.ldd + n] ? v * g.drop_scale : 0.f;
        if (g.drop_p > 0.f && ok) {
          unsigned long long z = drop_base + (unsigned long long)((long)m * g.N + n);
          z += 0x9E3779B97F4A7C15ull;
          z = (z ^ (z >> 30)) * 0xBF58476D1CE4E5B9ull;
          z = (z ^ (z >> 27)) * 0x94D049BB133111EBull;
          z ^= z >> 31;
          const float u = (float)(z >> 40) * (1.0f / 16777216.0f);
          v = u >= g.drop_p ? v * g.drop_scale : 0.f;
        }
        if (ref_staged) {
          v = bf16_bits_to_f32(stile[lrow * WTN + j * TS + r]) > 0.f ? v * g.ref_scale : 0.f;
        } else if (ref_staged2) {
          v = bf16_bits_to_f32(stile2[lrow * WTN + j * TS + r]) > 0.f ? v * g.ref_scale : 0.f;
        } else if (g.ref && ok) {
          const float rv = g.ref_bf16 ? bf16_bits_to_f32(((const unsigned short*)g.ref)[(long)m * g.ldr + n])
                                      : ((const float*)g.ref)[(long)m * g.ldr + n];
          v = rv > 0.f ? v * g.ref_scale : 0.f;
        }
        if (ok) vmax = max(vmax, absbits(v));
        if (staged) { stile[lrow * WTN + j * TS + r] = f32_to_bf16_bits(v); continue; }
        if (!ok) continue;
        const long o = (long)m * g.ldc + n;
        if (g.slab_stride > 0) __builtin_nontemporal_store(v, (float*)g.C + o + (long)zsplit * g.slab_stride);
        else if (g.atomic) atomicAdd((float*)g.C + o, v);
        else if (g.out_bf16) __builtin_nontemporal_store(f32_to_bf16_bits(v), (unsigned short*)g.C + o);
        else __builtin_nontemporal_store(v, (float*)g.C + o);
      }
    }
  if (staged) {
    constexpr int CPRW = WTN / 8;
#pragma unroll
    for (int q = 0; q < (WTM * CPRW) / 64; ++q) {
      const int idx = q * 64 + lane, lrow = idx / CPRW, ch = idx % CPRW;
      const int m = m0 + wm * WTM + lrow, n = n0t + wn * WTN + ch * 8;
      if (m < g.M && n < g.N) {
        __builtin_nontemporal_store(*(const u32x4*)(stile + lrow * WTN + ch * 8), (u32x4*)((unsigned short*)g.C + (long)m * g.ldc + n));
      }
    }
  }
  }
  if (g.absmax) {
    vmax = wave_reduce_max_u32(vmax);
    if (lane == 0) atomicMax((unsigned int*)g.absmax, vmax);
  }
}

template <typename T, int AMODE, int BMODE, int BM, int BN, int STAGES, int WTM, int WTN>
__global__ __launch_bounds__((BM / WTM) * (BN / WTN) * 64, 1) void gemm2_kernel(GemmArgs g) {
  extern __shared__ __attribute__((aligned(16))) char smem[];
  const int vgrid = (g.vgrid > 0 && gridDim.z == 1) ? g.vgrid : (int)gridDim.x;
  for (int vbid = blockIdx.x; vbid < vgrid; vbid += gridDim.x) {
  int bm, bn, zsplit = 0;
  if (gridDim.z > 1) {
    const int ntv = gridDim.x, tot = ntv * (int)gridDim.z;
    const int f = blockIdx.z * ntv + blockIdx.x;
    const int x = f & 7, j = f >> 3;
    const int w = x * (tot >> 3) + min(x, tot & 7) + j;
    zsplit = w / ntv;
    const int t = w - zsplit * ntv;
    bm = t % g.tiles_m; bn = t / g.tiles_m;
  } else {
    const int nwg = vgrid;
    const int bid = vbid;
    const int swz = (bid & 7) * (nwg >> 3) + (bid >> 3);
    const int patch = swz >> 6, within = swz & 63;
    const int pml = g.patch_m_log2;
    bm = ((patch % g.patches_m) << pml) + (within & ((1 << pml) - 1));
    bn = ((patch / g.patches_m) << (6 - pml)) + (within >> pml);
    if (bm >= g.tiles_m || bn >= g.tiles_n) continue;
  }
  gemm2_tile<T, AMODE, BMODE, BM, BN, STAGES, WTM, WTN>(g, bm, bn, zsplit, smem);
  if (vbid + (int)gridDim.x < vgrid) __syncthreads();
  }
}

struct GroupedProblem {
  const void* A; const void* B; float* C;
  int M, N, K, cH, cW, cC, cDil, k_per_split, nsplit, tiles_m, tiles_n;
  unsigned a_bytes, b_bytes;
  int lda, ldb;
};
constexpr int GROUPED_MAX = 40;
struct GroupedArgs {
  int n_problems, n_items;
  int first_item[GROUPED_MAX + 1];
  GroupedProblem p[GROUPED_MAX];
};

template <typename T, int BMODE = OP_CONV_B>
__global__ __launch_bounds__(1024, 1) void gemm2_grouped_kernel(GroupedArgs ga) {
  extern __shared__ __attribute__((aligned(16))) char smem[];
  const int G = gridDim.x;
  for (int vbid = blockIdx.x; vbid < ga.n_items; vbid += G) {
    const int round = vbid / G, within = vbid - round * G;
    const int in_round = min(G, ga.n_items - round * G);
    const int x = within & 7, j = within >> 3;
    const int per = in_round >> 3, extra = in_round & 7;
    if (j >= per + (x < extra ? 1 : 0)) continue;
    const int t = round * G + x * per + min(x, extra) + j;
    int pi = 0;
    while (pi + 1 < ga.n_problems && t >= ga.first_item[pi + 1]) ++pi;
    const GroupedProblem& P = ga.p[pi];
    const int local = t - ga.first_item[pi];
    const int ntile = P.tiles_m * P.tiles_n;
    const int zsplit = local / ntile, tl = local - zsplit * ntile;
    GemmArgs g = {};
    g.A = P.A; g.B = P.B; g.C = P.C; g.M = P.M; g.N = P.N; g.K = P.K; g.lda = P.lda; g.ldb = P.ldb; g.ldc = P.N;
    g.cH = P.cH; g.cW = P.cW; g.cC = P.cC; g.cDil = P.cDil; g.k_per_split = P.k_per_split;
    g.tiles_m = P.tiles_m; g.tiles_n = P.tiles_n; g.a_bytes = P.a_bytes; g.b_bytes = P.b_bytes;
    g.slab_stride = (long)P.M * P.N; g.drop_scale = 1.f; g.ref_scale = 1.f;
    gemm2_tile<T, OP_KSTRIDED, BMODE, 256, 256, 2, 64, 64>(g, tl % P.tiles_m, tl / P.tiles_m, zsplit, smem);
    __syncthreads();
  }
}


template <typename T, int AMODE, int BMODE, int BM, int BN, int STAGES, int WTM = 64, int WTN = 64>
int launch2(GemmArgs& g, int splitk, hipStream_t stream) {
  constexpr int BK = GT<T>::BK;
// ... 124 lines not shown
      for (int t = 0; t < 4; ++t) x[t] = __fmul_rn(x[t], sc); }
    if (f.bias) {
#pragma unroll
      for (int t = 0; t < 4; ++t) x[t] += f.bias[n + t]; }
    if (f.res) {
      if (f.res_bf16) { const unsigned short* p = (const unsigned short*)f.res + m * f.ldres + n;
#pragma unroll
        for (int t = 0; t < 4; ++t) x[t] += bf16_bits_to_f32(p[t]); }
      else { const f32x4 v = *(const f32x4*)((const float*)f.res + m * f.ldres + n);
#pragma unroll
        for (int t = 0; t < 4; ++t) x[t] += v[t]; }
    }
    if (f.relu) {
#pragma unroll
      for (int t = 0; t < 4; ++t) x[t] = relu_keep_nan(x[t]); }
    if (f.ref) {
#pragma unroll
      for (int t = 0; t < 4; ++t) {
        const float rv = f.ref_bf16 ? bf16_bits_to_f32(((const unsigned short*)f.ref)[m * f.ldr + n + t]) : ((const float*)f.ref)[m * f.ldr + n + t];
        x[t] = rv > 0.f ? x[t] * f.ref_scale : 0.f;
      }
    }
    if (f.out_bf16) {
      unsigned int w0 = (unsigned)f32_to_bf16_bits(x[0]) | ((unsigned)f32_to_bf16_bits(x[1]) << 16);
      unsigned int w1 = (unsigned)f32_to_bf16_bits(x[2]) | ((unsigned)f32_to_bf16_bits(x[3]) << 16);
      unsigned int* d = (unsigned int*)((unsigned short*)f.C + m * f.ldc + n);
      d[0] = w0; d[1] = w1;
    } else {
      f32x4 o = {x[0], x[1], x[2], x[3]};
      *(f32x4*)((float*)f.C + m * f.ldc + n) = o;
    }
  }
}

bool peel_geometry(int M, int N, int* r_out, long* sk_out) {
  const long tm = (M + 255) / 256, tn = (N + 255) / 256, tiles = tm * tn;
  if (!(tiles >= 512 && (tiles % 256) != 0 && (tiles % 256) <= 160)) return false;
  int r = 0;
  for (int c = 1; c <= 4 && !r; ++c)
    if (tn - c >= 2 && (tm * (tn - c)) % 256 == 0) r = c;
  if (!r) return false;
  const int N2 = N - (int)((tn - r) * 256);
  const long t128 = ((M + 127) / 128) * ((N2 + 127) / 128);
  long sk = 512 / t128;
  sk = sk < 1 ? 1 : (sk > 8 ? 8 : sk);
  while (sk > 1 && tm * r * sk >= 200) --sk;
  *r_out = r; *sk_out = sk;
  return true;
}

int effective_splits(int dtype, int K, int splitk) {
  const int bk = dtype == SW_BF16 ? 64 : 32;
  if (splitk < 1) splitk = 1;
  int kps = (K + splitk - 1) / splitk;
  kps = ((kps + bk - 1) / bk) * bk;
  return (K + kps - 1) / kps;
}

int check_align(const void* p) { return (((uintptr_t)p) & 15) ? -4 : 0; }

}

int sw_sgd_tile_t_block(int rows, int cols, float* param, const float* grad, float* buf, long ld_src, float lr, float wd, int first,
                        float mom, float gscale, unsigned short* st0, long ld0, unsigned short* st1, long ld1, const float* hyper,
                        hipStream_t stream);

static bool sgd_fused_shape_ok(int dtype, int a_kstrided, int b_kstrided, int M, int N, int K) {
  if (dtype != SW_BF16 || a_kstrided) return false;
  (void)b_kstrided;
  if ((M % 64) || (N % 64) || (K % 64) || K < 1024 || N <= 128) return false;
  return ((long)((M + 255) / 256) * ((N + 255) / 256)) >= 200;
}
static bool sgd_fused_accepts(int dtype, int a_kstrided, int b_kstrided, int M, int N, int K) {
  if (!sgd_fused_shape_ok(dtype, a_kstrided, b_kstrided, M, N, K)) return false;
  int r = 0; long sk = 1;
  if (!peel_geometry(M, N, &r, &sk)) return true;
  const int N1 = (int)(((N + 255) / 256 - r) * 256);
  return sgd_fused_shape_ok(dtype, a_kstrided, b_kstrided, M, N1, K) && ((N - N1) % 64) == 0;
}
extern "C" int sw_gemm_sgd_fused_supported(int dtype, int a_kstrided, int b_kstrided, int M, int N, int K) {
  return sgd_fused_accepts(dtype, a_kstrided, b_kstrided, M, N, K) ? 1 : 0;
}

extern "C" int sw_gemm(int dtype, int a_kstrided, int b_kstrided, int M, int N, int K, const void* A, long lda,
                       const void* B, long ldb, void* C, long ldc, const sw_epilogue* ep, int splitk,
                       hipStream_t stream) {
  SW_ENTER();
  if (M <= 0 || N <= 0 || K <= 0) return 0;
  const int epc = dtype == SW_BF16 ? 8 : 4;
  if (dtype != SW_BF16 && dtype != SW_F32) return -1;
  if (check_align(A) || check_align(B)) return -4;
  if ((lda % epc) || (ldb % epc)) return -5;
  if (!a_kstrided && (K % epc)) return -5;
  if (!b_kstrided && (K % epc)) return -5;
  if (a_kstrided && (M % epc)) return -5;
  if (b_kstrided && (N % epc)) return -5;
  if (a_kstrided && !b_kstrided) return -3;
  const bool plain = (!ep || (ep->out_dtype == SW_F32 && !ep->bias && !ep->relu && !ep->drop_mask && !(ep->drop_hash_p > 0.f) && !ep->relu_ref &&
                              !ep->accumulate_atomic && !ep->absmax_out && !ep->residual));
  const bool has_row_scale = ep && ep->fold_row_scale;
  float* const det_ws = (ep && plain) ? ep->splitk_workspace : nullptr;
  {
    int r = 0; long sk = 1;
    if (plain && !has_row_scale && splitk <= 1 && peel_geometry(M, N, &r, &sk)) {
      const long es = dtype == SW_BF16 ? 2 : 4;
      const long tn = (N + 255) / 256;
      const int N1 = (int)((tn - r) * 256), N2 = N - N1;
      const char* B2 = (const char*)B + (b_kstrided ? (long)N1 * es : (long)N1 * ldb * es);
      sw_epilogue ep1 = {};
      ep1.out_dtype = SW_F32; ep1.drop_scale = 1.f; ep1.ref_scale = 1.f;
      const sw_sgd_tensor* fz = ep ? ep->sgd_fused : nullptr;
      if (fz) {
        if (!sgd_fused_accepts(dtype, a_kstrided, b_kstrided, M, N, K) || !fz->stage1) return -5;
        ep1.sgd_fused = fz; ep1.sgd_momentum = ep->sgd_momentum; ep1.sgd_grad_scale = ep->sgd_grad_scale;
      }
      int rc = sw_gemm(dtype, a_kstrided, b_kstrided, M, N1, K, A, lda, B, ldb, C, ldc, &ep1, 1, stream);
      if (rc) return rc;
      float* C2 = (float*)C + N1;
      ep1.sgd_fused = nullptr;
      sw_epilogue ep2 = ep1;
      if (det_ws) ep2.splitk_workspace = det_ws;
      else if (sk > 1) {
        hipError_t e = hipMemset2DAsync(C2, (size_t)ldc * 4, 0, (size_t)N2 * 4, (size_t)M, stream);
        if (e != hipSuccess) return (int)e;
        ep2.accumulate_atomic = 1;
      }
      rc = sw_gemm(dtype, a_kstrided, b_kstrided, M, N2, K, A, lda, B2, ldb, C2, ldc, &ep2, (int)sk, stream);
      if (rc || !fz) return rc;
      return sw_sgd_tile_t_block(M, N2, fz->param + N1, C2, fz->momentum_buf + N1, ldc, fz->lr, fz->weight_decay, fz->first_step,
                                 ep->sgd_momentum, ep->sgd_grad_scale, fz->stage0 ? (unsigned short*)fz->stage0 + N1 : nullptr, fz->ld0,
                                 (unsigned short*)fz->stage1 + (long)N1 * fz->ld1, fz->ld1, fz->hyper_dev, stream);
    }
  }
  if (ep && ep->sgd_fused) {
    const sw_sgd_tensor* fz = ep->sgd_fused;
    if (!plain || splitk > 1 || !sgd_fused_accepts(dtype, a_kstrided, b_kstrided, M, N, K)) return -5;
    if (fz->stage_kind != 3 || fz->stage_dtype != SW_BF16 || !fz->stage1 || fz->d0 < N || !fz->param || !fz->momentum_buf) return -5;
    if ((ldc % 4) || (fz->ld0 % 4) || (fz->ld1 % 8) || ((((uintptr_t)fz->param) | ((uintptr_t)fz->momentum_buf)) & 15) ||
        (((uintptr_t)fz->stage0) & 7) || (((uintptr_t)fz->stage1) & 15)) return -4;
  }
  const int eff = effective_splits(dtype, K, splitk);
  const bool fold_ep = ep && !plain && (eff > 1 || (ep->fold_row_scale && ep->residual)) && ep->splitk_workspace &&
                       !ep->accumulate_atomic && !ep->drop_mask && !(ep->drop_hash_p > 0.f) && !ep->absmax_out;
  if (fold_ep) {
    if ((N % 4) || (ldc % 4) || (((uintptr_t)C) & 7) || (((uintptr_t)ep->splitk_workspace) & 15)) return -5;
    if (ep->residual && ((ep->ld_res % 4) || (((uintptr_t)ep->residual) & 7))) return -5;
    float* const slabs = ep->splitk_workspace;
    GemmArgs gs = {};
    gs.A = A; gs.B = B; gs.M = M; gs.N = N; gs.K = K; gs.lda = lda; gs.ldb = ldb;
    gs.C = slabs; gs.ldc = N; gs.slab_stride = (long)M * N; gs.drop_scale = 1.f; gs.ref_scale = 1.f;
    {
      const long es = dtype == SW_BF16 ? 2 : 4;
      const long ab = (long)(a_kstrided ? K : M) * lda * es, bb = (long)(b_kstrided ? K : N) * ldb * es;
      if (ab >= 0xFFFFFF00L || bb >= 0xFFFFFF00L) return -6;
      gs.a_bytes = (unsigned)ab; gs.b_bytes = (unsigned)bb;
    }
    const int am = a_kstrided ? OP_KSTRIDED : OP_KCONTIG, bmo = b_kstrided ? OP_KSTRIDED : OP_KCONTIG;
    const int rc = dtype == SW_BF16 ? dispatch_modes<unsigned short>(gs, am, bmo, eff, stream) : dispatch_modes<float>(gs, am, bmo, eff, stream);
    if (rc) return rc;
    FoldEp f = {};
    f.M = M; f.N = N; f.nslab = eff; f.ws = slabs; f.C = C; f.ldc = ldc; f.out_bf16 = ep->out_dtype == SW_BF16;
    f.bias = ep->bias; f.row_scale = ep->fold_row_scale;
    f.res = ep->residual; f.ldres = ep->ld_res; f.res_bf16 = ep->res_dtype == SW_BF16;
    f.relu = ep->relu; f.ref = ep->relu_ref; f.ldr = ep->ld_ref; f.ref_bf16 = ep->ref_dtype == SW_BF16; f.ref_scale = ep->ref_scale;
    long blocks = (((long)M * N >> 2) + 255) / 256;
    blocks = blocks < 1 ? 1 : (blocks > 4096 ? 4096 : blocks);
    hipLaunchKernelGGL(splitk_fold_ep_kernel, dim3((unsigned)blocks), dim3(256), 0, stream, f);
    SW_CHECK_LAUNCH();
    return 0;
  }
  const bool det = det_ws != nullptr && eff > 1;
  if (det && (((uintptr_t)det_ws) & 15)) return -4;
  GemmArgs g = {};
  g.A = A; g.B = B; g.C = C; g.M = M; g.N = N; g.K = K; g.lda = lda; g.ldb = ldb; g.ldc = ldc;
  if (ep) {
    g.bias = ep->bias; g.drop = ep->drop_mask; g.ldd = ep->ld_drop; g.drop_scale = ep->drop_scale;
    g.ref = ep->relu_ref; g.ldr = ep->ld_ref; g.ref_scale = ep->ref_scale; g.ref_bf16 = ep->ref_dtype == SW_BF16;
    g.res = ep->residual; g.ldres = ep->ld_res; g.res_bf16 = ep->res_dtype == SW_BF16;
    g.relu = ep->relu; g.out_bf16 = ep->out_dtype == SW_BF16; g.atomic = ep->accumulate_atomic; g.absmax = ep->absmax_out;
    if (ep->sgd_fused) {
      const sw_sgd_tensor* fz = ep->sgd_fused;
      g.sgd_param = fz->param; g.sgd_mom = fz->momentum_buf; g.sgd_ld = ldc;
      g.sgd_st0 = (unsigned short*)fz->stage0; g.sgd_ld0 = fz->ld0; g.sgd_st1 = (unsigned short*)fz->stage1; g.sgd_ld1 = fz->ld1;
      g.sgd_hyper = fz->hyper_dev; g.sgd_lr = fz->lr; g.sgd_wd = fz->weight_decay; g.sgd_first = fz->first_step;
      g.sgd_momentum = ep->sgd_momentum; g.sgd_gscale = ep->sgd_grad_scale;
    }
    if (!ep->drop_mask && ep->drop_hash_p > 0.f) {
      unsigned long long x = ep->drop_seed;
      x += 0x9E3779B97F4A7C15ull;
      x = (x ^ (x >> 30)) * 0xBF58476D1CE4E5B9ull;
      x = (x ^ (x >> 27)) * 0x94D049BB133111EBull;
      x ^= x >> 31;
      g.drop_seed_mixed = x; g.drop_offset = ep->drop_offset; g.drop_p = ep->drop_hash_p;
      g.drop_offset_dev = (const unsigned long long*)ep->drop_offset_dev;
    }
  }
  {
    const long es = dtype == SW_BF16 ? 2 : 4;
    const long ab = (long)(a_kstrided ? K : M) * lda * es, bb = (long)(b_kstrided ? K : N) * ldb * es;
    if (ab >= 0xFFFFFF00L || bb >= 0xFFFFFF00L) return -6;
    g.a_bytes = (unsigned)ab; g.b_bytes = (unsigned)bb;
  }
  const int am = a_kstrided ? OP_KSTRIDED : OP_KCONTIG, bmo = b_kstrided ? OP_KSTRIDED : OP_KCONTIG;
  if (det) {
    g.C = det_ws; g.ldc = N; g.slab_stride = (long)M * N; g.atomic = 0;
  }
  const int rc = dtype == SW_BF16 ? dispatch_modes<unsigned short>(g, am, bmo, det ? eff : splitk, stream)
                                  : dispatch_modes<float>(g, am, bmo, det ? eff : splitk, stream);
  if (rc) return rc;
  if (!det) {
    if (ep && ep->fold_row_scale) {
      if (!plain || ep->out_dtype != SW_F32) return -5;
      long blocks = ((long)M * N + 255) / 256;
      blocks = blocks > 4096 ? 4096 : blocks;
      hipLaunchKernelGGL(scale_rows_kernel, dim3((unsigned)blocks), dim3(256), 0, stream, M, N, (float*)C, ldc, ep->fold_row_scale);
      SW_CHECK_LAUNCH();
    }
    return 0;
  }
  const int vec = ((N % 4) == 0 && (ldc % 4) == 0 && (((uintptr_t)C) & 15) == 0) ? 1 : 0;
  long blocks = (((long)M * N >> (vec ? 2 : 0)) + 255) / 256;
  blocks = blocks < 1 ? 1 : (blocks > 4096 ? 4096 : blocks);
  hipLaunchKernelGGL(splitk_reduce_kernel, dim3((unsigned)blocks), dim3(256), 0, stream, M, N, eff, det_ws, (float*)C, ldc, vec,
                     ep ? ep->fold_row_scale : nullptr);
  SW_CHECK_LAUNCH();
  return 0;
}

extern "C" long sw_gemm_splitk_workspace_floats(int M, int N, int K, int splitk) {
  if (M <= 0 || N <= 0 || K <= 0) return 0;
  if (splitk > 1) return (long)splitk * M * N;
  int r = 0; long sk = 1;
  if (peel_geometry(M, N, &r, &sk) && sk > 1) {
    const long tn = (N + 255) / 256;
    const int N2 = N - (int)((tn - r) * 256);
    return sk * (long)M * N2;
  }
  return 0;
}

int sw_conv3x3_direct_try(int nimg, int H, int W, int Cin, int Cout, int dilation, const void* in, const void* wk, void* out,
                          const sw_epilogue* ep, hipStream_t stream);

extern "C" int sw_conv3x3_igemm(int dtype, int nimg, int H, int W, int Cin, int Cout, int dilation, const void* in,
                                const void* wk, void* out, const sw_epilogue* ep, hipStream_t stream) {
  SW_ENTER();
  const int epc = dtype == SW_BF16 ? 8 : 4;
  if (dtype != SW_BF16 && dtype != SW_F32) return -1;
  if (Cin % epc) return -5;
  if (check_align(in) || check_align(wk)) return -4;
  if (dtype == SW_BF16) {
    const int rc = sw_conv3x3_direct_try(nimg, H, W, Cin, Cout, dilation, in, wk, out, ep, stream);
    if (rc != 0) return rc < 0 ? -rc : 0;
  }
  GemmArgs g = {};
  g.A = in; g.B = wk; g.C = out; g.M = nimg * H * W; g.N = Cout; g.K = 9 * Cin; g.lda = 0; g.ldb = 9L * Cin; g.ldc = Cout;
  g.cH = H; g.cW = W; g.cC = Cin; g.cDil = dilation;
  g.krot = dtype == SW_BF16 ? 1 : 0;
  if (ep) {
    g.bias = ep->bias; g.drop = ep->drop_mask; g.ldd = ep->ld_drop; g.drop_scale = ep->drop_scale;
    g.ref = ep->relu_ref; g.ldr = ep->ld_ref; g.ref_scale = ep->ref_scale; g.ref_bf16 = ep->ref_dtype == SW_BF16;
    g.relu = ep->relu; g.out_bf16 = ep->out_dtype == SW_BF16; g.atomic = ep->accumulate_atomic;
  }
  {
    const long es = dtype == SW_BF16 ? 2 : 4;
    const long ab = (long)nimg * H * W * Cin * es, bb = (long)Cout * 9 * Cin * es;
    if (ab >= 0xFFFFFF00L || bb >= 0xFFFFFF00L) return -6;
    g.a_bytes = (unsigned)ab; g.b_bytes = (unsigned)bb;
  }
  const int bk = dtype == SW_BF16 ? 64 : 32;
  const int amode = (Cin % bk == 0) ? OP_CONV_A : OP_CONV_A_GEN;
  return dtype == SW_BF16 ? dispatch_modes<unsigned short>(g, amode, OP_KCONTIG, 1, stream)
                          : dispatch_modes<float>(g, amode, OP_KCONTIG, 1, stream);
}

namespace {
__device__ __forceinline__ void wgrad_reduce_body(int Cout, int Cin, int nslab, const float* __restrict__ slabs,
                                                  float* __restrict__ out, int co, int parts, int part, float* s_t,
                                                  const float* __restrict__ cout_scale = nullptr, const int accumulate = 0) {
  const int CI = Cin / parts, ci0 = part * CI;
  const int cv = CI >> 2, nv = 9 * cv;
  const long slab_f = (long)Cout * 9 * Cin;
  const float* src = slabs + (long)co * 9 * Cin + ci0;
  for (int q = threadIdx.x; q < nv; q += 256) {
    const int tap = q / cv, c4 = q - tap * cv;
    const float* p = src + (long)tap * Cin + c4 * 4;
    f32x4 a0 = {0.f, 0.f, 0.f, 0.f}, a1 = a0, a2 = a0, a3 = a0;
    int z = 0;
    for (; z + 8 <= nslab; z += 8) {
      f32x4 v[8];
#pragma unroll
      for (int u = 0; u < 8; ++u) v[u] = *(const f32x4*)(p + (long)(z + u) * slab_f);
      a0 += v[0]; a1 += v[1]; a2 += v[2]; a3 += v[3];
      a0 += v[4]; a1 += v[5]; a2 += v[6]; a3 += v[7];
    }
    for (; z < nslab; ++z) a0 += *(const f32x4*)(p + (long)z * slab_f);
    f32x4 r = (a0 + a1) + (a2 + a3);
    if (cout_scale) { const float sc = cout_scale[co]; r[0] = __fmul_rn(r[0], sc); r[1] = __fmul_rn(r[1], sc); r[2] = __fmul_rn(r[2], sc); r[3] = __fmul_rn(r[3], sc); }
    *(f32x4*)(s_t + tap * CI + c4 * 4) = r;
  }
  __syncthreads();
  f32x4* dst = (f32x4*)(out + ((long)co * Cin + ci0) * 9);
  for (int q = threadIdx.x; q < nv; q += 256) {
    f32x4 o;
#pragma unroll
    for (int j = 0; j < 4; ++j) {
      const int e = 4 * q + j, ci = e / 9, tap = e - 9 * ci;
      o[j] = s_t[tap * CI + ci];
    }
    if (accumulate) o += dst[q];
    dst[q] = o;
  }
}

__global__ __launch_bounds__(256) void wgrad_reduce_kernel(int Cout, int Cin, int nslab, const float* __restrict__ slabs,
                                                           float* __restrict__ out, const float* __restrict__ cout_scale, int accumulate) {
  extern __shared__ __attribute__((aligned(16))) float s_t[];
  wgrad_reduce_body(Cout, Cin, nslab, slabs, out, blockIdx.x, (int)gridDim.y, blockIdx.y, s_t, cout_scale, accumulate);
}

constexpr int FOLD_MAX = 32;
struct FoldMulti {
  int n;
  int first_wg[FOLD_MAX + 1];
  int Cin[FOLD_MAX], Cout[FOLD_MAX], nslab[FOLD_MAX], parts[FOLD_MAX];
  const float* ws[FOLD_MAX];
  float* out[FOLD_MAX];
};
__global__ __launch_bounds__(256) void wgrad_reduce_multi_kernel(FoldMulti f) {
  extern __shared__ __attribute__((aligned(16))) float s_t[];
  int i = 0;
  while (i + 1 < f.n && (int)blockIdx.x >= f.first_wg[i + 1]) ++i;
  const int local = blockIdx.x - f.first_wg[i];
  wgrad_reduce_body(f.Cout[i], f.Cin[i], f.nslab[i], f.ws[i], f.out[i], local / f.parts[i], f.parts[i], local % f.parts[i], s_t);
}

}
// ... 266 lines not shown
```

### sos-wsod_amd/ops.py

```python
import ctypes

import torch

from ._lib import SW_BF16, SW_F32, Epilogue, check, lib


def _p(t):
    return None if t is None else ctypes.c_void_p(t.data_ptr())


def _floats(vals, n):
    return (ctypes.c_float * n)(*[float(v) for v in vals])


def _workspace256(nbytes, device):
    ws = torch.empty(nbytes + 256, device=device, dtype=torch.uint8)
    return ws, ctypes.c_void_p((ws.data_ptr() + 255) // 256 * 256)


_raw_stream = getattr(torch._C, "_cuda_getCurrentRawStream", None)


def _stream():
    if _raw_stream is not None:
# ... 65 lines not shown

    def __enter__(self):
        import gc
        gc.collect()
        self._was = gc.isenabled()
        gc.disable()
        return self

    def __exit__(self, *exc):
        import gc
        if self._was:
            gc.enable()
        return False


class grad_scope:

    def __enter__(self):
        global GRAD_SCOPE
        self._prev, GRAD_SCOPE = GRAD_SCOPE, self
        self.bufs, self.uses, self.queued = {}, {}, {}
        return self

    def finish(self):
        left = [k for k, q in self.queued.items() if q["probs"]]
        if left:
            self.bufs, self.uses, self.queued = {}, {}, {}
            raise RuntimeError(f"grad_scope: {len(left)} queued weight gradient(s) were never finished — a use counted in the forward pass "
                               "did not take part in backward(); run this graph without ops.grad_scope")

    def __exit__(self, exc_type, *exc):
        global GRAD_SCOPE
        GRAD_SCOPE = self._prev
        left = [k for k, q in self.queued.items() if q["probs"]]
        self.bufs, self.uses, self.queued = {}, {}, {}
        if left and exc_type is None:
            raise RuntimeError(f"grad_scope: {len(left)} queued weight gradient(s) were never finished — a use counted in the forward pass "
                               "did not take part in backward(); run this graph without ops.grad_scope")
        return False


CALLER_GRAD_ENABLED = True


class CountedFunction(torch.autograd.Function):

    @classmethod
    def apply(cls, *args, **kwargs):
        global CALLER_GRAD_ENABLED
        prev, CALLER_GRAD_ENABLED = CALLER_GRAD_ENABLED, torch.is_grad_enabled()
        try:
            return super().apply(*args, **kwargs)
        finally:
            CALLER_GRAD_ENABLED = prev


def count_use(key):
    if GRAD_SCOPE is not None and key is not None and CALLER_GRAD_ENABLED:
        GRAD_SCOPE.uses[key] = GRAD_SCOPE.uses.get(key, 0) + 1


def pending_grad(key, shape):
    if GRAD_SCOPE is None or key is None:
        return None
    buf = GRAD_SCOPE.bufs.get(key)
    if buf is None or buf.numel() != int(torch.Size(shape).numel()) or not buf.is_contiguous():
        return None
    return buf.view(shape)


def note_grad(key, buf):
    if GRAD_SCOPE is not None and key is not None:
        GRAD_SCOPE.bufs[key] = buf.view(buf.shape)


def grad_target(param, shape, dev):
    view = param.__dict__.get("_sw_grad_view")
    if (view is not None and param.grad is None and tuple(view.shape) == tuple(shape) and view.device == dev
            and view.dtype == torch.float32 and view.is_contiguous()):
        return view.detach()
    return torch.empty(*shape, device=dev, dtype=torch.float32)


def _launch(tag, fn):
    if TIMER is None or tag is None:
        return fn()
    return TIMER.wrap(tag, fn)


def _need_gpu(*ts):
    for t in ts:
        if t is not None and not t.is_cuda:
            raise RuntimeError("sos-wsod_amd kernels need GPU tensors (there is no CPU fallback)")


def make_epilogue(bias=None, relu=False, drop_mask=None, drop_scale=2.0, relu_ref=None, ref_scale=1.0,
                  out_dtype=torch.float32, atomic=False, absmax_out=None, drop_hash=None, splitk_workspace=None, residual=None,
                  row_scale=None):
    ep = Epilogue()
    ep.bias = None if bias is None else bias.data_ptr()
    ep.relu = int(relu)
    ep.drop_mask = None if drop_mask is None else drop_mask.data_ptr()
    ep.ld_drop = 0 if drop_mask is None else drop_mask.stride(0)
    ep.drop_scale = float(drop_scale)
    if relu_ref is not None and relu_ref.dim() != 2:
        raise ValueError("relu_ref: a (rows, columns) matrix (its row pitch is the reference's leading dimension)")
    ep.relu_ref = None if relu_ref is None else relu_ref.data_ptr()
    ep.ld_ref = 0 if relu_ref is None else relu_ref.stride(0)
    ep.ref_scale = float(ref_scale)
    ep.ref_dtype = SW_F32 if relu_ref is None else dt(relu_ref)
    ep.out_dtype = dt(out_dtype)
    ep.accumulate_atomic = int(atomic)
    ep.absmax_out = None if absmax_out is None else absmax_out.data_ptr()
    ep.splitk_workspace = None if splitk_workspace is None else splitk_workspace.data_ptr()
    if drop_hash is not None and drop_mask is None:
        ep.drop_seed, ep.drop_offset, ep.drop_hash_p = int(drop_hash[0]) & (2 ** 64 - 1), int(drop_hash[1]), float(drop_hash[2])
        if len(drop_hash) > 3 and drop_hash[3] is not None:
            ep.drop_offset_dev = drop_hash[3].data_ptr()
    if residual is not None and residual.dim() != 2:
        raise ValueError("residual: a (rows, columns) matrix")
    ep.residual = None if residual is None else residual.data_ptr()
    ep.ld_res = 0 if residual is None else residual.stride(0)
    ep.res_dtype = SW_F32 if residual is None else dt(residual)
    ep.fold_row_scale = None if row_scale is None else row_scale.data_ptr()
    ep._keepalive = (bias, drop_mask, relu_ref, absmax_out, splitk_workspace, drop_hash, residual, row_scale)
    return ep


def gemm(A, B, C, M, N, K, a_kstrided=False, b_kstrided=False, lda=None, ldb=None, ldc=None, ep=None, splitk=1, tag=None):
    _need_gpu(A, B, C)
    lda = A.stride(0) if lda is None else lda
    ldb = B.stride(0) if ldb is None else ldb
    ldc = C.stride(0) if ldc is None else ldc
    if ep is None:
        ep = make_epilogue(out_dtype=C.dtype)
    if (C.dtype == torch.float32 or splitk > 1) and not ep.accumulate_atomic and not ep.splitk_workspace:
        need = int(lib.sw_gemm_splitk_workspace_floats(M, N, K, splitk))
        if need > 0:
            ws = torch.empty(need, device=C.device, dtype=torch.float32)
            ep.splitk_workspace = ws.data_ptr()
            ep._keepalive = ep._keepalive + (ws,)
    check(_launch(tag, lambda: lib.sw_gemm(dt(A), int(a_kstrided), int(b_kstrided), M, N, K, _p(A), lda, _p(B), ldb, _p(C),
                                           ldc, ctypes.byref(ep), splitk, _stream())), "sw_gemm")
    return C


def conv3x3(x, wk, out, dilation, ep, tag=None):
    _need_gpu(x, wk, out)
    n, H, W, Cin = x.shape
    Cout = out.shape[3]
    if TIMER is not None and tag is not None:
        TIMER.note(tag, 2.0 * n * H * W * Cout * 9 * Cin)
    check(_launch(tag, lambda: lib.sw_conv3x3_igemm(dt(x), n, H, W, Cin, Cout, dilation, _p(x), _p(wk), _p(out),
                                                    ctypes.byref(ep), _stream())), "sw_conv3x3_igemm")
    return out


def conv3x3_relu_pool2(x, wk, bias, out_pooled, tag=None):
    _need_gpu(x, wk, out_pooled)
    n, H, W, Cin = x.shape
    Cout = out_pooled.shape[3]
    if TIMER is not None and tag is not None:
        TIMER.note(tag, 2.0 * n * H * W * Cout * 9 * Cin)
    rc = _launch(tag, lambda: lib.sw_conv3x3_relu_pool2(dt(x), n, H, W, Cin, Cout, _p(x), _p(wk), _p(bias), _p(out_pooled), _stream()))
    if rc < 0:
        check(rc, "sw_conv3x3_relu_pool2")
    return rc == 1


def conv3x3_multi(problems):
    from ._lib import ConvProblem
    n = len(problems)
    if n == 0:
        return
    if 1 < n <= 8 and problems[0][0].dtype == torch.bfloat16:
        arr = (ConvProblem * n)()
        for i, (x, wk, out, ep) in enumerate(problems):
            _need_gpu(x, wk, out)
            q = arr[i]
            q.nimg, q.H, q.W, q.Cin = x.shape
            q.Cout = out.shape[3]
            q.in_, q.wk, q.out, q.ep = x.data_ptr(), wk.data_ptr(), out.data_ptr(), ctypes.pointer(ep)
        rc = int(lib.sw_conv3x3_multi(SW_BF16, n, arr, _stream()))
        if rc == 1:
            return
        if rc < 0:
            check(rc, "sw_conv3x3_multi")
    for x, wk, out, ep in problems:
        conv3x3(x, wk, out, 1, ep)


def conv3x3_wgrad(x, dy, dw_oihw, dilation, splitk=1, workspace=None, tag=None, cout_scale=None, accumulate=False):
    _need_gpu(x, dy, dw_oihw)
    n, H, W, Cin = x.shape
    Cout = dy.shape[3]
    need = int(lib.sw_conv3x3_wgrad_workspace_floats(dt(x), n, H, W, Cin, Cout, splitk))
    if workspace is None or workspace.numel() < need:
        workspace = torch.empty(need, device=x.device, dtype=torch.float32)
    check(_launch(tag, lambda: lib.sw_conv3x3_wgrad(dt(x), n, H, W, Cin, Cout, dilation, _p(x), _p(dy), _p(dw_oihw),
                                                    _p(workspace), splitk, _p(cout_scale), int(accumulate), _stream())), "sw_conv3x3_wgrad")
    return dw_oihw


def conv3x3_wgrad_small(x, dy, dw_oihw, cout_scale=None, accumulate=False):
    _need_gpu(x, dy, dw_oihw)
    n, H, W, Cin = x.shape
    check(lib.sw_conv3x3_wgrad_small(dt(x), n, H, W, Cin, dy.shape[3], _p(x), _p(dy), _p(cout_scale), _p(dw_oihw), int(accumulate),
                                     _stream()), "sw_conv3x3_wgrad_small")
    return dw_oihw


def conv3x3_wgrad_nslab(x, cout, splitk):
    n, H, W, Cin = x.shape
    return int(lib.sw_conv3x3_wgrad_workspace_floats(dt(x), n, H, W, Cin, cout, splitk)) // (cout * 9 * Cin)


def conv3x3_wgrad_nslab_shape(dtype, n, H, W, Cin, cout, splitk):
    code = SW_BF16 if dtype == torch.bfloat16 else SW_F32
    return int(lib.sw_conv3x3_wgrad_workspace_floats(code, n, H, W, Cin, cout, splitk)) // (cout * 9 * Cin)


def conv3x3_wgrad_grouped(problems, tag=None):
    from ._lib import WgradProblem
    n = len(problems)
    if n == 0:
        return
    arr = (WgradProblem * n)()
    for i, (x, dy, slabs, dil, nsplit) in enumerate(problems):
        _need_gpu(x, dy, slabs)
        q = arr[i]
        q.nimg, q.H, q.W, q.Cin = x.shape
        q.Cout, q.dilation, q.nsplit = dy.shape[3], int(dil), int(nsplit)
        q.x, q.dy, q.slabs = x.data_ptr(), dy.data_ptr(), slabs.data_ptr()
    if TIMER is not None and tag is not None:
        TIMER.note(tag, sum(2.0 * x.numel() * 9 * dy.shape[3] for x, dy, _, _, _ in problems))
    check(_launch(tag, lambda: lib.sw_conv3x3_wgrad_grouped(dt(problems[0][0]), n, arr, _stream())), "sw_conv3x3_wgrad_grouped")


# ... 140 lines not shown


def _argmax_bits(argmax):
    if argmax.dtype == torch.int32:
        return 32
    if argmax.dtype in (torch.int16, torch.uint16):
        return 16
    raise TypeError(f"ROIPool argmax must be int32 or (u)int16, got {argmax.dtype}")


def roi_argmax_dtype(H, W):
    return torch.int16 if H * W < 65535 else torch.int32


def argmax_to_int32(argmax):
    if argmax.dtype == torch.int32:
        return argmax
    a = argmax.view(torch.int16).to(torch.int32) & 0xFFFF
    return torch.where(a == 0xFFFF, torch.full_like(a, -1), a)


def absmax(x, out=None):
    if out is None:
        out = torch.empty(1, device=x.device, dtype=torch.float32)
    check(lib.sw_absmax(dt(x), x.numel(), _p(x), _p(out), _stream()), "sw_absmax")
    return out


def roi_pool_bwd(dout, argmax, rois, dfeat, PH, PW, row_scale=None, row_scale_add=0.0, relu_ref=None, dout_absmax="auto",
                 tag=None, spatial_scale=0.0):
    _need_gpu(dout, argmax, rois, dfeat)
    n, H, W, C = dfeat.shape
    R = rois.shape[0]
    if isinstance(dout_absmax, str):
        dout_absmax = absmax(dout)
    check(_launch(tag, lambda: lib.sw_roi_pool_bwd(dt(dfeat), n, H, W, C, PH, PW, _p(dout), _p(argmax), _argmax_bits(argmax),
                                                   _roi_pitch(dout, argmax), _p(rois), R, _p(row_scale), float(row_scale_add),
                                                   _p(relu_ref), _p(dout_absmax), _p(dfeat), float(spatial_scale), _stream())),
          "sw_roi_pool_bwd")
    return dfeat


def wsddn_mil(logits, V, R, K, cls_col, det_col, gt_onehot, scores, loss_view, dlogits=None, grad_scale=None,
              mean_scores=None, workspace=None):
    _need_gpu(logits, gt_onehot, scores, loss_view)
    if workspace is None:
        workspace = torch.empty(int(lib.sw_wsddn_workspace_floats(V, R, K)), device=logits.device, dtype=torch.float32)
    check(lib.sw_wsddn_mil(V, R, K, _p(logits), logits.stride(0), cls_col, det_col, _p(gt_onehot), _p(scores),
                           _p(loss_view), _p(dlogits), 0 if dlogits is None else dlogits.stride(0), _p(grad_scale),
                           _p(mean_scores), 0 if mean_scores is None else mean_scores.stride(-2), _p(workspace),
                           _stream()), "sw_wsddn_mil")


def sgd_multi(entries, momentum, grad_scale=1.0):
    from ._lib import SgdTensor
    n = len(entries)
    if n == 0:
        return
    arr = (SgdTensor * n)()
    for i, e in enumerate(entries):
        _fill_sgd_tensor(arr[i], e)
    check(lib.sw_sgd_multi(n, arr, float(momentum), float(grad_scale), _stream()), "sw_sgd_multi")


def _fill_sgd_tensor(d, e):
    p = e["param"]
    g = e.get("grad")
    d.param, d.grad, d.momentum_buf, d.n = p.data_ptr(), (None if g is None else g.data_ptr()), e["buf"].data_ptr(), p.numel()
    d.lr, d.weight_decay, d.first_step = float(e["lr"]), float(e["weight_decay"]), int(e["first"])
    hy = e.get("hyper")
    d.hyper_dev = None if hy is None else hy.data_ptr()
    st = e.get("staging")
    if st is None:
        d.stage_kind = 0
    else:
        d.stage_kind, d.stage_dtype = st["kind"], dt(st["dtype"])
        d.stage0 = None if st["stage0"] is None else st["stage0"].data_ptr()
        d.stage1 = None if st["stage1"] is None else st["stage1"].data_ptr()
        d.d0, d.d1, d.d2, d.ld0, d.ld1 = st["d0"], st["d1"], st["d2"], st["ld0"], st.get("ld1", 0)


def gemm_sgd_fused_supported(dtype, M, N, K, a_kstrided=False, b_kstrided=False):
    return bool(lib.sw_gemm_sgd_fused_supported(dt(dtype), int(a_kstrided), int(b_kstrided), int(M), int(N), int(K)))


def attach_sgd_fused(ep, entry, momentum, grad_scale=1.0):
    from ._lib import SgdTensor
    d = SgdTensor()
    _fill_sgd_tensor(d, entry)
    ep.sgd_fused = ctypes.addressof(d)
    ep.sgd_momentum, ep.sgd_grad_scale = float(momentum), float(grad_scale)
    ep._keepalive = ep._keepalive + (d, entry["param"], entry["buf"], entry.get("hyper"))
    return ep


def mean_views(x, out):
    V = x.shape[0]
    check(lib.sw_mean_views(V, out.numel(), _p(x), _p(out), _stream()), "sw_mean_views")
    return out


def oicr_mean_probs(logits, V, R, K, n_rounds, cls_col0, col_stride, out):
    _need_gpu(logits, out)
    check(lib.sw_oicr_mean_probs(V, R, K, n_rounds, _p(logits), logits.stride(0), cls_col0, col_stride, _p(out), _stream()),
          "sw_oicr_mean_probs")
    return out


def mine_workspace_bytes(R, top_k, G, n_rounds=1):
    return int(lib.sw_mine_workspace_bytes(R, top_k, G)) * n_rounds


def oicr_mine_label(scores, gt_classes_i32, boxes, K, top_k, thresh, nms_thresh, iou_bg, iou_fg, lab_class, lab_weight,
                    lab_index, pgt_count, pgt_index, pgt_class, pgt_score, workspace):
    _need_gpu(scores, gt_classes_i32, boxes)
    n_rounds = 1 if scores.dim() == 2 else scores.shape[0]
    R, ncol = scores.shape[-2:]
    G = gt_classes_i32.numel()
    _launch("mine_label", lambda: check(
        lib.sw_oicr_mine_label(R, ncol, K, n_rounds, _p(scores), _p(gt_classes_i32), G, _p(boxes), int(top_k),
                               float(thresh), float(nms_thresh), float(iou_bg), float(iou_fg), _p(lab_class),
                               _p(lab_weight), _p(lab_index), _p(pgt_count), _p(pgt_index), _p(pgt_class), _p(pgt_score),
                               _p(workspace), _stream()), "sw_oicr_mine_label"))


def oicr_refine_loss(logits, V, R, K, cls_col, box_col, boxes, lab_class, lab_weight, lab_index, pred_view, reg_weights,
                     loss_view, dlogits=None, grad_scale=None, workspace=None, n_rounds=1, col_stride=0):
    rw = _floats(reg_weights, 4)
    if workspace is None:
        workspace = torch.empty(n_rounds * 2 * V * R, device=logits.device, dtype=torch.float32)
    check(lib.sw_oicr_refine_loss(V, R, K, n_rounds, _p(logits), logits.stride(0), cls_col, box_col, col_stride, _p(boxes),
                                  _p(lab_class), _p(lab_weight), _p(lab_index), _p(pred_view), rw, _p(loss_view),
                                  _p(dlogits), 0 if dlogits is None else dlogits.stride(0), _p(grad_scale), _p(workspace),
                                  _stream()), "sw_oicr_refine_loss")


def colsum(X, M, N, out, ld=None, accumulate=False):
    need = int(lib.sw_colsum_workspace_floats(dt(X), M, N))
    ws = torch.empty(max(need, 4), device=X.device, dtype=torch.float32)
    check(lib.sw_colsum(dt(X), M, N, _p(X), X.stride(0) if ld is None else ld, _p(out), _p(ws), int(accumulate), _stream()), "sw_colsum")
    return out


def convert_2d(src_f32, dst, rows, cols, ld_src=None, ld_dst=None):
    check(lib.sw_convert_2d(dt(dst), rows, cols, _p(src_f32), src_f32.stride(0) if ld_src is None else ld_src, _p(dst),
                            dst.stride(0) if ld_dst is None else ld_dst, _stream()), "sw_convert_2d")
    return dst


def split_bf16x3(src_f32, side, along_rows=False, out=None):
    _need_gpu(src_f32)
    rows, cols = src_f32.shape
    assert src_f32.dtype == torch.float32 and src_f32.stride(1) == 1
    shape = (6 * rows, cols) if along_rows else (rows, 6 * cols)
    if out is None or tuple(out.shape) != shape:
        out = torch.empty(shape[0], shape[1] + 128, device=src_f32.device, dtype=torch.bfloat16)[:, :shape[1]]
    check(lib.sw_split_bf16x3(rows, cols, _p(src_f32), src_f32.stride(0), _p(out), out.stride(0), int(side), int(bool(along_rows)), _stream()),
          "sw_split_bf16x3")
    return out


def gemm_f32x3(A, B, C, M, N, K, a_kstrided=False, b_kstrided=False, ep=None, tag=None, A3=None, B3=None):
    if A3 is None:
        A3 = split_bf16x3(A, 0, along_rows=a_kstrided)
    if B3 is None:
        B3 = split_bf16x3(B, 1, along_rows=b_kstrided)
# ... 731 lines not shown
```

### sos-wsod_amd/roi_heads_oicrplus.py

```python
from typing import Dict, List

import os
import numpy as np
import torch
import torch.nn as nn

from . import ops, staging
from .box_head import DiscriminativeAdaptionNeck
from .events import get_event_storage, has_event_storage
from .fast_rcnn_oicr import OICROutputLayers
from .fast_rcnn_wsddn import WSDDNOutputLayers
from .poolers import ROIPooler
from .registry import ROI_BOX_HEAD_REGISTRY, ROI_HEADS_REGISTRY
from .structures import ShapeSpec

LOSS_NAMES_FMT = ["loss_cls"]


def get_image_level_gt(targets, num_classes):
    if targets is None:
        return None, None, None
    cls, ints, ohs = [], [], []
    for t in targets:
        g = t.gt_classes
# ... 392 lines not shown
        n_loss = 1 + 2 * RK
        K1 = K + 1
        col_stride = 5 * K + 1
        loss_view = torch.empty(B, n_loss, V, device=dev, dtype=torch.float32)
        dlogits = torch.empty(M, LD, device=dev, dtype=torch.float32) if inp["need_grad"] else None
        ones = inp["ones"]
        images = []
        for b in range(B):
            R, off, G = Rs[b], offs[b], inp["G"][b]
            lg = logits[off:off + V * R]
            dl = None if dlogits is None else dlogits[off:off + V * R]
            scores = torch.empty(V, R, K, device=dev, dtype=torch.float32)
            mine_scores = torch.empty(RK, R, K1, device=dev, dtype=torch.float32)
            ops.wsddn_mil(lg, V, R, K, cols["cls"], cols["det"], inp["gt_onehot"][b], scores, loss_view[b, 0], dl, ones,
                          mean_scores=mine_scores[0])
            if RK > 1:
                ops.oicr_mean_probs(lg, V, R, K, RK - 1, cols["cls_score0"], col_stride, mine_scores[1:])
            top_k = max(int(R * self.mist_p), 1)
            ws = torch.empty(ops.mine_workspace_bytes(R, top_k, G, RK), device=dev, dtype=torch.uint8)
            lab_c = torch.empty(RK, R, device=dev, dtype=torch.int32); lab_w = torch.empty(RK, R, device=dev, dtype=torch.float32)
            lab_i = torch.empty(RK, R, device=dev, dtype=torch.int32); cnt = torch.empty(RK, device=dev, dtype=torch.int32)
            pi = torch.empty(RK, top_k * G, device=dev, dtype=torch.int32); pc = torch.empty_like(pi)
            ps = torch.empty(RK, top_k * G, device=dev, dtype=torch.float32)
            boxes = inp["boxes"][b]
            ops.oicr_mine_label(mine_scores, inp["gt_int32"][b], boxes[0], K, top_k, self.mist_thre, 0.01,
                                self.iou_thresholds[0], self.iou_thresholds[1], lab_c, lab_w, lab_i, cnt, pi, pc, ps, ws)
            ops.oicr_refine_loss(lg, V, R, K, cols["cls_score0"], cols["bbox_pred0"], boxes, lab_c, lab_w, lab_i,
                                 inp["pred_view"], self.bbox_reg_weights, loss_view[b, 1:], dl, ones, n_rounds=RK,
                                 col_stride=col_stride)
            images.append({"scores": scores, "mine_scores": mine_scores, "fc7": h2[off:off + V * R], "logits": lg,
                           "rounds": [dict(lab_class=lab_c[k], lab_weight=lab_w[k], lab_index=lab_i[k],
                                           pgt_count=cnt[k:k + 1], pgt_index=pi[k], pgt_class=pc[k], pgt_score=ps[k])
                                      for k in range(RK)]})
        out = torch.empty(n_loss + 2, device=dev, dtype=torch.float32)
        losses, total, finite = out[:n_loss], out[n_loss:n_loss + 1], out[n_loss + 1:]
        ops.loss_finalize(loss_view, losses, out[n_loss:])
        aux = dict(images[0])
        aux["images"] = images
        self.last_aux = aux
        self._last_finite = finite
        return dict(losses=losses, total=total, feats=feats, pooled=pooled, argmax=argmax, h1=h1, h2=h2, W1=W1, W1T=W1T, W2=W2,
                    W2T=W2T, Wh=Wh, dlogits=dlogits, inp=inp, train_dropout=training_dropout)

    def _col_to_loss(self, device):
        K = self.num_classes
        idx = torch.zeros(self.ld_head, dtype=torch.int32)
        idx[: 2 * K] = 0
        for k in range(self.refine_K):
            base = 2 * K + k * (5 * K + 1)
            idx[base: base + K + 1] = 1 + 2 * k
            idx[base + K + 1: base + 5 * K + 1] = 2 + 2 * k
        return idx.to(device)

    def _handle(self, device, fresh=False):
        if fresh:
            return torch.empty(1, device=device, dtype=torch.float32)
        z = getattr(self, "_zero_handle", None)
        if z is None or z.device != device:
            z = self._zero_handle = torch.zeros(1, device=device, dtype=torch.float32)
        return z

    def _train_backward_top(self, st, params_top, g_losses, g_total):
        dt_ = self.compute_dtype
        inp = st["inp"]
        B, M = inp["B"], inp["M"]
        LD = self.ld_head
        pooled, h1, h2, W2, Wh = st["pooled"], st["h1"], st["h2"], st["W2"], st["Wh"]
        dev = pooled.device
        D1, D2 = h1.shape[1], h2.shape[1]
        if not hasattr(self, "_c2l") or self._c2l.device != dev:
            self._c2l = self._col_to_loss(dev)
        if g_losses is not None:
            g_losses = g_losses.contiguous().float()
        if g_total is not None:
            g_total = g_total.contiguous().float()
        dl = torch.empty(M, LD, device=dev, dtype=dt_)
        ops.scale_cols_loss(st["dlogits"], g_losses, g_total, self._c2l, 1.0 / B, dl, M, LD, self.n_head_cols)
        rs = 2.0 if st["train_dropout"] else 1.0
        dbh = torch.empty(LD, device=dev, dtype=torch.float32); ops.colsum(dl, M, LD, dbh)
        dWh = torch.empty(LD, D2, device=dev, dtype=torch.float32)
        ops.gemm(dl, h2, dWh, LD, D2, M, a_kstrided=True, b_kstrided=True, splitk=4)
        dz2 = _padded(M, D2, dev, dt_)
        WhT = self._head_weights_t(Wh, dev)
        if WhT is not None:
            ops.gemm(dl, WhT, dz2, M, D2, LD, ep=ops.make_epilogue(relu_ref=h2, ref_scale=rs, out_dtype=dt_))
        else:
            ops.gemm(dl, Wh, dz2, M, D2, LD, b_kstrided=True, ep=ops.make_epilogue(relu_ref=h2, ref_scale=rs, out_dtype=dt_))
        db2 = ops.grad_target(self.box_head.fc2.bias, (D2,), dev); ops.colsum(dz2, M, D2, db2)
        epc = 8 if dt_ == torch.bfloat16 else 4
        wgrad_nn = M % epc == 0

        def dz_t(dz, D):
            return ops.transpose_2d(dz, torch.empty(D, M + 8 * epc, device=dev, dtype=dt_)[:, :M], M, D)
        dW2 = ops.grad_target(self.box_head.fc2.weight, (D2, D1), dev)
        if wgrad_nn:
            self._fc_gemm(dz_t(dz2, D2), h1, dW2, D2, D1, M, b_kstrided=True)
        else:
            ops.gemm(dz2, h1, dW2, D2, D1, M, a_kstrided=True, b_kstrided=True)
        dz1 = _padded(M, D1, dev, dt_)
        if st.get("W2T") is not None:
            self._fc_gemm(dz2, st["W2T"], dz1, M, D1, D2, ep=ops.make_epilogue(relu_ref=h1, ref_scale=rs, out_dtype=dt_),
                          wname="fc2T", wmaster=self.box_head.fc2.weight)
        else:
            ops.gemm(dz2, W2, dz1, M, D1, D2, b_kstrided=True, ep=ops.make_epilogue(relu_ref=h1, ref_scale=rs, out_dtype=dt_))
        st["dz1"] = dz1
        dparams = [dW2, db2]
        row = 0
        for i in range(2, len(params_top), 2):
            n = params_top[i].shape[0]
            dparams += [dWh[row:row + n], dbh[row:row + n]]
            row += n
        return [g if p.requires_grad else None for g, p in zip(dparams, params_top)]

    def _fused_fc1_plan(self, M, D0, D1):
        opt = getattr(self, "_fused_opt", None)
        if (opt is None or self.compute_dtype != torch.bfloat16 or (M % 8) or getattr(self, "fp32x3", False)
                or getattr(self, "_fc6_panels", None) is not None or getattr(self, "_staged", False)
                or not ops.gemm_sgd_fused_supported(torch.bfloat16, D1, D0, M, False, True)):
            return None
        w = self.box_head.fc1.weight
        if not w.requires_grad or w.grad is not None:
            return None
        return opt.fused_update_entry(w)

    def _fused_fc1_wgrad(self, st):
        plan = st.pop("fused_fc1")
        entry, momentum, finish = plan
        pooled, dz1 = st["pooled"], st["dz1"]
        dev, M = pooled.device, st["inp"]["M"]
        D0, D1 = pooled.shape[1], dz1.shape[1]

        def nn():
            dzt = ops.transpose_2d(dz1, torch.empty(D1, M + 64, device=dev, dtype=torch.bfloat16)[:, :M], M, D1)
            scratch = torch.empty(D1, D0, device=dev, dtype=torch.float32)
            ep = ops.attach_sgd_fused(ops.make_epilogue(out_dtype=torch.float32), entry, momentum, 1.0)
            ops.gemm(dzt, pooled, scratch, D1, D0, M, b_kstrided=True, ep=ep)
        ops._launch("fc6_wgrad_sgd", nn)
        finish()

    def _train_backward_fc6(self, st, defer_fused=False):
        dt_ = self.compute_dtype
        pooled, dz1 = st["pooled"], st["dz1"]
        dev, M = pooled.device, st["inp"]["M"]
        D0, D1 = pooled.shape[1], dz1.shape[1]
        epc = 8 if dt_ == torch.bfloat16 else 4
        db1 = ops.grad_target(self.box_head.fc1.bias, (D1,), dev); ops.colsum(dz1, M, D1, db1)
        plan = self._fused_fc1_plan(M, D0, D1)
        if plan is not None:
            st["fused_fc1"] = plan
            if not defer_fused:
                self._fused_fc1_wgrad(st)
            return None, db1
        dW1 = ops.grad_target(self.box_head.fc1.weight, (D1, D0), dev)
        panels = getattr(self, "_fc6_panels", None)
        if panels is not None and panels[0] > 1 and D1 % (256 * panels[0]) == 0:
            rows = D1 // panels[0]
            dzt = ops.transpose_2d(dz1, torch.empty(D1, M + 8 * epc, device=dev, dtype=dt_)[:, :M], M, D1) if M % epc == 0 else None
            for i in range(panels[0]):
                if dzt is not None:
                    ops.gemm(dzt[i * rows:(i + 1) * rows], pooled, dW1[i * rows:(i + 1) * rows], rows, D0, M, b_kstrided=True)
                else:
                    ops.gemm(dz1[:, i * rows:(i + 1) * rows], pooled, dW1[i * rows:(i + 1) * rows], rows, D0, M, a_kstrided=True, b_kstrided=True)
                panels[1](i, dW1[i * rows:(i + 1) * rows])
        elif M % epc == 0:
            def nn():
                dzt = ops.transpose_2d(dz1, torch.empty(D1, M + 8 * epc, device=dev, dtype=dt_)[:, :M], M, D1)
                self._fc_gemm(dzt, pooled, dW1, D1, D0, M, b_kstrided=True)
            ops._launch("fc6_wgrad", nn)
        else:
            ops.gemm(dz1, pooled, dW1, D1, D0, M, a_kstrided=True, b_kstrided=True, tag="fc6_wgrad")
        return dW1, db1

    def _train_backward_pool(self, st, feat_req):
        dt_ = self.compute_dtype
        inp = st["inp"]
        B, Rs, offs, M = inp["B"], inp["R"], inp["off"], inp["M"]
        pooled, dz1, W1 = st["pooled"], st["dz1"], st["W1"]
        dev = pooled.device
        D0, D1 = pooled.shape[1], dz1.shape[1]
        dfeats = [None] * len(feat_req)
        if any(feat_req):
            dpooled = _padded(M, D0, dev, dt_, pad=64)
            amax = ops.fill_zero(torch.empty(1, device=dev, dtype=torch.float32))
            if st["W1T"] is not None:
                self._fc_gemm(dz1, st["W1T"], dpooled, M, D0, D1, ep=ops.make_epilogue(out_dtype=dt_, absmax_out=amax),
                              tag="fc6_dgrad", wname="fc1T", wmaster=self.box_head.fc1.weight)
            else:
                ops.gemm(dz1, W1, dpooled, M, D0, D1, b_kstrided=True, ep=ops.make_epilogue(out_dtype=dt_, absmax_out=amax),
                         tag="fc6_dgrad")
            P = self.box_pooler.output_size
            for b in range(B):
                R, off = Rs[b], offs[b]
                for s in range(2):
                    if not feat_req[2 * b + s]:
                        continue
                    f = st["feats"][2 * b + s]
                    df = torch.empty_like(f)
                    r0 = off + 2 * s * R
                    ops.roi_pool_bwd(dpooled[r0:r0 + 2 * R], st["argmax"][r0:r0 + 2 * R], inp["rois"][b][s], df, P, P,
                                     row_scale=inp["obj"][b][2 * s:2 * s + 2].reshape(-1), row_scale_add=1.0, relu_ref=f,
                                     dout_absmax=amax, tag="roi_bwd", spatial_scale=self.box_pooler.scale)
                    dfeats[2 * b + s] = df
        if "fused_fc1" in st:
            self._fused_fc1_wgrad(st)
        return dfeats

    def _prepare_inputs(self, proposals_list, targets1, device, need_grad):
        K = self.num_classes
        B = len(proposals_list[0])
        assert B >= 1 and all(len(p) == B for p in proposals_list)
        _, gt_ints, gt_oh = get_image_level_gt(targets1, K)
        if not hasattr(self, "_consts") or self._consts[0].device != device:
            self._consts = (torch.ones(max(2, 2 * self.refine_K), device=device),
                            torch.tensor([0, 1, 2, 2], dtype=torch.int32, device=device))
        Rs, Gs, offs, boxes, obj, rois = [], [], [], [], [], []
        off = 0
        for b in range(B):
            props = [p[b] for p in proposals_list]
            R = len(props[0])
            assert all(len(p) == R for p in props), "the 4 proposal sets are index aligned (dataset_mapper.py:353-361)"
            bl = [p.proposal_boxes.tensor.to(device=device, dtype=torch.float32).contiguous() for p in props]
            ol = [p.objectness_logits.to(device=device, dtype=torch.float32).contiguous() for p in props]
            bx = torch.empty(4, R, 4, device=device, dtype=torch.float32)
            ob = torch.empty(4, R, device=device, dtype=torch.float32)
            ro = torch.empty(2, 2 * R, 5, device=device, dtype=torch.float32)
            if device.type == "cuda":
                ops.pack_views(bl, ol, bx, ob, ro)
            else:
                bx.copy_(torch.stack(bl)); ob.copy_(torch.stack(ol))
                ro[..., 1:] = bx.view(2, 2 * R, 4); ro[:, :R, 0] = 0; ro[:, R:, 0] = 1
            Rs.append(R); Gs.append(int(gt_ints[b].numel())); offs.append(off); boxes.append(bx); obj.append(ob); rois.append(ro)
            off += 4 * R
        nG = sum(Gs)
        if self._prestaged_labels is not None:
            devbuf, staged_G = self._prestaged_labels
            assert tuple(staged_G) == tuple(Gs), "the class counts are kernel arguments of the captured step"
        elif device.type == "cuda":
            host = torch.empty(nG + B * K, dtype=torch.float32, pin_memory=True)
            self._fill_label_host(host, gt_ints, gt_oh, nG)
            devbuf = host.to(device, non_blocking=True)
        else:
            devbuf = torch.cat([torch.cat(gt_ints).to(torch.int32).view(torch.float32), gt_oh.reshape(-1)])
        gt_i32, gt_onehot, g0 = [], [], 0
        for b in range(B):
            gt_i32.append(devbuf[g0:g0 + Gs[b]].view(torch.int32)); g0 += Gs[b]
            gt_onehot.append(devbuf[nG + b * K: nG + (b + 1) * K])
        return dict(B=B, R=Rs, G=Gs, off=offs, M=off, boxes=boxes, obj=obj, rois=rois, gt_int32=gt_i32, gt_onehot=gt_onehot,
                    ones=self._consts[0], pred_view=self._consts[1], need_grad=need_grad)

# ... 56 lines not shown
```

Baseline: 502.7 images/s.

## Fuse bias-grad column sums and transposed output into GEMM and conv epilogues

Adds colsum_part and out_t side outputs to the GEMM and direct-conv epilogues. The fc7/fc6 backward GEMMs now write per-tile column partial sums and a transposed bf16 copy of dz. This removes the separate colsum and transpose_2d passes used for the bias gradients and the NN weight-grad layout. Conv backward-data kernels likewise emit partial column sums for the previous layer's bias gradient, replacing deferred colsum reads of dz. The cost is extra epilogue work, LDS exchange and syncs in those kernels, plus partial-sum buffers that still need a fold kernel.

```diff
diff --git a/include/soswsod_hip.h b/include/soswsod_hip.h
--- a/include/soswsod_hip.h
+++ b/include/soswsod_hip.h
@@ -37,14 +37,19 @@
   const float* fold_row_scale;
   const struct sw_sgd_tensor_s* sgd_fused;
   float sgd_momentum, sgd_grad_scale;
+  float* colsum_part;
+  void* out_t;
+  long ld_t;
 } sw_epilogue;
 
 int sw_gemm(int dtype, int a_kstrided, int b_kstrided, int M, int N, int K, const void* A, long lda, const void* B,
             long ldb, void* C, long ldc, const sw_epilogue* ep, int splitk, sw_stream_t stream);
+int sw_gemm_side_output_parts(int dtype, int a_kstrided, int b_kstrided, int M, int N, int K);
 long sw_gemm_splitk_workspace_floats(int M, int N, int K, int splitk);
 
 int sw_conv3x3_igemm(int dtype, int nimg, int H, int W, int Cin, int Cout, int dilation, const void* in,
                      const void* wk, void* out, const sw_epilogue* ep, sw_stream_t stream);
+int sw_conv3x3_colsum_parts(int dtype, int nimg, int H, int W, int Cin, int Cout, int dilation);
 int sw_conv3x3_relu_pool2(int dtype, int nimg, int H, int W, int Cin, int Cout, const void* in, const void* wk, const float* bias,
                           void* out_pooled, sw_stream_t stream);
 typedef struct sw_conv_problem {
diff --git a/sos-wsod_amd/_lib.py b/sos-wsod_amd/_lib.py
--- a/sos-wsod_amd/_lib.py
+++ b/sos-wsod_amd/_lib.py
@@ -22,6 +22,7 @@
         ("residual", c_void_p), ("ld_res", c_long), ("res_dtype", c_int),
         ("fold_row_scale", c_void_p),
         ("sgd_fused", c_void_p), ("sgd_momentum", c_float), ("sgd_grad_scale", c_float),
+        ("colsum_part", c_void_p), ("out_t", c_void_p), ("ld_t", c_long),
     ]
 
 
@@ -98,9 +99,11 @@
     "sw_gemm": (c_int, [c_int, c_int, c_int, c_int, c_int, c_int, c_void_p, c_long, c_void_p, c_long, c_void_p, c_long,
                         _EP, c_int, c_void_p]),
     "sw_gemm_splitk_workspace_floats": (c_long, [c_int, c_int, c_int, c_int]),
+    "sw_gemm_side_output_parts": (c_int, [c_int, c_int, c_int, c_int, c_int, c_int]),
     "sw_gemm_sgd_fused_supported": (c_int, [c_int, c_int, c_int, c_int, c_int, c_int]),
     "sw_conv3x3_igemm": (c_int, [c_int, c_int, c_int, c_int, c_int, c_int, c_int, c_void_p, c_void_p, c_void_p, _EP,
                                  c_void_p]),
+    "sw_conv3x3_colsum_parts": (c_int, [c_int, c_int, c_int, c_int, c_int, c_int, c_int]),
     "sw_conv3x3_wgrad": (c_int, [c_int, c_int, c_int, c_int, c_int, c_int, c_int, c_void_p, c_void_p, c_void_p, c_void_p,
                                  c_int, c_void_p, c_int, c_void_p]),
     "sw_conv3x3_wgrad_workspace_floats": (c_long, [c_int, c_int, c_int, c_int, c_int, c_int, c_int]),
diff --git a/sos-wsod_amd/backbone_vgg.py b/sos-wsod_amd/backbone_vgg.py
--- a/sos-wsod_amd/backbone_vgg.py
+++ b/sos-wsod_amd/backbone_vgg.py
@@ -240,19 +240,23 @@
                 w = params[pidx]
                 if w.requires_grad:
                     cout = blk.out_channels
-                    slab_off, row_off, nslab, nrow, splits = {}, {}, 0, 0, {}
+                    slab_off, row_off, nslab, nrow, splits, side_rows = {}, {}, 0, 0, {}, {}
                     for i in live:
                         x_in = infos[i][si][0][ci][0]
                         n, H, W, cin = x_in.shape
+                        side_rows[i] = 0
+                        if (ops.FUSED_SIDE_OUTPUTS and ci + 1 < blk.num_conv and dtype == torch.bfloat16
+                                and not module.x3_layer(dtype, cout, cout)):
+                            side_rows[i] = ops.conv3x3_colsum_parts(dtype, n, H, W, cout, cout, blk.dilation)
                         splits[i] = (direct_ns[(pidx, i)] if direct_ns is not None
                                      else _wgrad_grouped_splits(nmul * n * H * W, bk, target))
                         slab_off[i], row_off[i] = nslab, nrow
                         nslab += ops.conv3x3_wgrad_nslab_shape(wdt, nmul * n, H, W, cin, cout, splits[i])
-                        nrow += ops.colsum_nrows(dtype, n * H * W, cout)
+                        nrow += side_rows[i] if side_rows[i] else ops.colsum_nrows(dtype, n * H * W, cout)
                     cin = infos[live[0]][si][0][ci][0].shape[3]
                     plan[pidx] = dict(ws=torch.empty(nslab, cout * 9 * cin, device=dev, dtype=torch.float32),
                                       rows=torch.empty(nrow, cout, device=dev, dtype=torch.float32), slab_off=slab_off,
-                                      row_off=row_off, nslab=nslab, nrow=nrow, splits=splits, cin=cin,
+                                      row_off=row_off, nslab=nslab, nrow=nrow, splits=splits, cin=cin, side_rows=side_rows,
                                       dw=ops.grad_target(w, (cout, cin, 3, 3), dev),
                                       db=ops.grad_target(params[pidx + 1], (cout,), dev))
                 if (si, ci) == first_trainable:
@@ -316,12 +320,15 @@
                         xw.record_stream(consumer_stream); dw_.record_stream(consumer_stream)
                         dz.record_stream(consumer_stream)
                     deferred.append((xw, dw_, pl["ws"][pl["slab_off"][i]:], blk.dilation, pl["splits"][i]))
-                    module._colsum_deferred.append((dz.view(npix, blk.out_channels), pl["rows"][pl["row_off"][i]:]))
+                    if not pl["side_rows"][i]:
+                        module._colsum_deferred.append((dz.view(npix, blk.out_channels), pl["rows"][pl["row_off"][i]:]))
                 if (si, ci) == first_trainable:
                     return
                 dx = torch.empty(n, H, W, cin, device=g.device, dtype=dtype)
                 ref = x_in.view(n * H * W, cin) if ci > 0 else None
-                epd = ops.make_epilogue(relu_ref=ref, out_dtype=dtype)
+                pl_in = plan.get(pidx - 2) if ci > 0 else None
+                cpart = pl_in["rows"][pl_in["row_off"][i]:] if (pl_in is not None and pl_in["side_rows"][i]) else None
+                epd = ops.make_epilogue(relu_ref=ref, out_dtype=dtype, colsum_part=cpart)
                 if module.x3_layer(dtype, blk.out_channels, cin):
                     cout = blk.out_channels
                     dz3 = ops.split_bf16x3(dz.view(n * H * W, cout), 0,
diff --git a/sos-wsod_amd/csrc/conv_direct.hip b/sos-wsod_amd/csrc/conv_direct.hip
--- a/sos-wsod_amd/csrc/conv_direct.hip
+++ b/sos-wsod_amd/csrc/conv_direct.hip
@@ -15,7 +15,35 @@
   int out_f32;
   int tiles_x, tiles_y, n_px_tiles, n_co_blocks, total;
   unsigned in_bytes, wk_bytes;
+  float* colsum_part;
 };
+
+template <int TN, int NW>
+__device__ __forceinline__ void direct_colsum_store(const float (&cs)[8], const int lane, const int wave, float* xw, float* ys,
+                                                    float* __restrict__ row, const int co0, const int Cout) {
+  constexpr int NG = 64 / (TN / 8);
+  const int grp = lane / (TN / 8), ch = lane % (TN / 8);
+  *(f32x4*)(xw + grp * TN + ch * 8) = f32x4{cs[0], cs[1], cs[2], cs[3]};
+  *(f32x4*)(xw + grp * TN + ch * 8 + 4) = f32x4{cs[4], cs[5], cs[6], cs[7]};
+  __builtin_amdgcn_s_waitcnt(0xc07f);
+  float sw = 0.f;
+  if (lane < TN) {
+#pragma unroll
+    for (int r = 0; r < NG; ++r) sw += xw[r * TN + lane];
+    ys[wave * TN + lane] = sw;
+  }
+  __syncthreads();
+  if (wave == 0 && lane < TN && co0 + lane < Cout) {
+    float tot = 0.f;
+#pragma unroll
+    for (int w = 0; w < NW; ++w) tot += ys[w * TN + lane];
+    row[co0 + lane] = tot;
+  }
+}
+__device__ __forceinline__ void direct_colsum_add(float (&cs)[8], const u32x4& v) {
+#pragma unroll
+  for (int t = 0; t < 4; ++t) { cs[2 * t] += __uint_as_float(v[t] << 16); cs[2 * t + 1] += __uint_as_float(v[t] & 0xFFFF0000u); }
+}
 
 template <int N> __device__ __forceinline__ void wait_vm() { asm volatile("s_waitcnt vmcnt(%0)" ::"n"(N) : "memory"); }
 
@@ -230,6 +258,9 @@
         }
     }
     __builtin_amdgcn_s_waitcnt(0xc07f);
+    float cs[8];
+#pragma unroll
+    for (int t = 0; t < 8; ++t) cs[t] = 0.f;
 #pragma unroll
     for (int it = 0; it < TN / 16; ++it) {
       const int idx = it * 64 + lane;
@@ -248,8 +279,12 @@
           }
         }
         *(u32x4*)(out + o) = v;
-      }
-    }
+        if (g.colsum_part) direct_colsum_add(cs, v);
+      }
+    }
+    if (g.colsum_part)
+      direct_colsum_store<TN, 8>(cs, lane, wave_all, (float*)S, (float*)(smem + 8 * 2 * NI * 64 * 16 + 8 * (32 * TN * 2)),
+                                 g.colsum_part + (long)px_tile * g.Cout, co0, g.Cout);
     return;
   }
   if (g.out_f32) {
@@ -321,6 +356,9 @@
     }
     return;
   }
+  float cs[8];
+#pragma unroll
+  for (int t = 0; t < 8; ++t) cs[t] = 0.f;
 #pragma unroll
   for (int it = 0; it < TN / 8; ++it) {
     const int idx = it * 64 + lane;
@@ -339,8 +377,11 @@
         }
       }
       *(u32x4*)(out + o) = v;
-    }
-  }
+      if (g.colsum_part) direct_colsum_add(cs, v);
+    }
+  }
+  if (g.colsum_part)
+    direct_colsum_store<TN, 4>(cs, lane, wave, (float*)S, (float*)(smem + 4 * (64 * TN * 2)), g.colsum_part + (long)px_tile * g.Cout, co0, g.Cout);
 }
 
 template <int DIL, int TN, int KG = 1>
@@ -431,6 +472,23 @@
   }
 }
 
+}
+
+namespace {
+void direct_form(int nimg, int H, int W, int Cin, int Cout, int* kg, int* tn) {
+  const int n_px_tiles = ((W + TW - 1) / TW) * ((H + TH - 1) / TH) * nimg;
+  const bool few = n_px_tiles * ((Cout + 63) / 64) <= 384;
+  *kg = (few && (Cin % (2 * CK)) == 0) ? 2 : 1;
+  *tn = (few && *kg == 1) ? 32 : 64;
+}
+}
+
+extern "C" int sw_conv3x3_colsum_parts(int dtype, int nimg, int H, int W, int Cin, int Cout, int dilation) {
+  if (dtype != SW_BF16 || nimg <= 0 || H <= 0 || W <= 0) return 0;
+  if ((Cin % CK) || Cin < 64 || (Cout % 8) || (dilation != 1 && dilation != 2)) return 0;
+  if ((long)nimg * H * W * Cin * 2 >= 0xFFFFFF00L || (long)Cout * 9 * Cin * 2 >= 0xFFFFFF00L) return 0;
+  const long rows = (long)((W + TW - 1) / TW) * ((H + TH - 1) / TH) * nimg;
+  return rows > 2147483647L ? 0 : (int)rows;
 }
 
 int sw_conv3x3_direct_try(int nimg, int H, int W, int Cin, int Cout, int dilation, const void* in, const void* wk, void* out,
@@ -456,12 +514,16 @@
   DirectArgs g = {};
   g.in = in; g.wk = wk; g.out = out; g.bias = ep->bias; g.ref = ep->relu_ref; g.relu = ep->relu;
   g.out_f32 = ep->out_dtype == SW_F32;
+  if (ep->colsum_part) {
+    if (g.out_f32) return 0;
+    if (((uintptr_t)ep->colsum_part) & 15) return -4;
+    g.colsum_part = ep->colsum_part;
+  }
   g.nimg = nimg; g.H = H; g.W = W; g.Cin = Cin; g.Cout = Cout;
   g.tiles_x = (W + TW - 1) / TW; g.tiles_y = (H + TH - 1) / TH;
   g.n_px_tiles = g.tiles_x * g.tiles_y * nimg;
-  const bool few = g.n_px_tiles * ((Cout + 63) / 64) <= 384;
-  const int kg = (few && (Cin % (2 * CK)) == 0) ? 2 : 1;
-  const int tn = (few && kg == 1) ? 32 : 64;
+  int kg, tn;
+  direct_form(nimg, H, W, Cin, Cout, &kg, &tn);
   g.n_co_blocks = (Cout + tn - 1) / tn;
   g.total = g.n_px_tiles * g.n_co_blocks;
   const long ib = (long)nimg * H * W * Cin * 2, wb = (long)Cout * 9 * Cin * 2;
@@ -532,6 +594,7 @@
     if (!ep || q.nimg <= 0 || q.H <= 0 || q.W <= 0) return 0;
     if ((q.Cin % CK) || q.Cin < 64 || (q.Cout % 8)) return 0;
     if (ep->out_dtype != SW_BF16 || ep->drop_mask || ep->accumulate_atomic || ep->absmax_out || (ep->drop_hash_p > 0.f) || ep->residual) return 0;
+    if (ep->colsum_part || ep->out_t) return 0;
     if (ep->relu_ref && (ep->ref_dtype != SW_BF16 || ep->ld_ref != q.Cout || ep->ref_scale != 1.0f)) return 0;
     if ((((uintptr_t)q.in | (uintptr_t)q.wk | (uintptr_t)q.out | (uintptr_t)ep->relu_ref) & 15)) return 0;
     DirectArgs& g = m.p[i];
diff --git a/sos-wsod_amd/csrc/gemm.hip b/sos-wsod_amd/csrc/gemm.hip
--- a/sos-wsod_amd/csrc/gemm.hip
+++ b/sos-wsod_amd/csrc/gemm.hip
@@ -27,6 +27,7 @@
   float* sgd_param; float* sgd_mom; long sgd_ld;
   unsigned short* sgd_st0; long sgd_ld0; unsigned short* sgd_st1; long sgd_ld1;
   const float* sgd_hyper; float sgd_lr, sgd_wd, sgd_momentum, sgd_gscale; int sgd_first;
+  float* colsum_part; unsigned short* out_t; long ld_t;
 };
 
 template <typename T> struct GT;
@@ -443,6 +444,10 @@
     if (g.sgd_param && g.sgd_hyper) { sgd_lr = g.sgd_hyper[0]; sgd_wd = g.sgd_hyper[1]; }
     __syncthreads();
     const bool vec_ok = g.staged_out;
+    const bool side_t = g.colsum_part || g.out_t;
+    float csum = 0.f;
+    constexpr int XS_OFF = NW * (32 * LDW) * 4 + NW * WTN * TP * 2;
+    static_assert(XS_OFF + NW * WTN * 4 <= STAGES * STAGE_BYTES, "column-sum exchange fits the ring");
     auto quarter = [&](auto qc) {
       constexpr int q = decltype(qc)::value;
       constexpr int NPC = (32 * (WTN / 4)) / 64;
@@ -556,14 +561,21 @@
             }
           } else {
             unsigned short* dst = (unsigned short*)g.C + o;
+            unsigned short hb[CP];
+#pragma unroll
+            for (int t = 0; t < CP; ++t) hb[t] = f32_to_bf16_bits(v[t]);
+            if (side_t) {
+#pragma unroll
+              for (int t = 0; t < CP; ++t) tT[(c0 + t) * TP + row] = hb[t];
+            }
             if (full && vec_ok) {
               u32x4 w;
 #pragma unroll
-              for (int t = 0; t < 4; ++t) w[t] = (unsigned)f32_to_bf16_bits(v[2 * t]) | ((unsigned)f32_to_bf16_bits(v[2 * t + 1]) << 16);
+              for (int t = 0; t < 4; ++t) w[t] = (unsigned)hb[2 * t] | ((unsigned)hb[2 * t + 1] << 16);
               __builtin_nontemporal_store(w, (u32x4*)dst);
             } else {
 #pragma unroll
-              for (int t = 0; t < CP; ++t) if (nb + t < g.N) dst[t] = f32_to_bf16_bits(v[t]);
+              for (int t = 0; t < CP; ++t) if (nb + t < g.N) dst[t] = hb[t];
             }
           }
         }
@@ -572,7 +584,24 @@
       const bool bf16_rows = g.out_bf16 && g.slab_stride <= 0 && !g.atomic;
       if (bf16_rows) { if (plain_ep) pieces(IntC<8>{}, IntC<1>{}); else pieces(IntC<8>{}, IntC<0>{}); }
       else { if (plain_ep) pieces(IntC<4>{}, IntC<1>{}); else pieces(IntC<4>{}, IntC<0>{}); }
-      if (g.sgd_param && g.sgd_st1) {
+      if (g.colsum_part) {
+        __builtin_amdgcn_s_waitcnt(0xc07f);
+        const int nvalid = g.M - (m0 + wm * WTM + q * 32);
+        float sq = 0.f;
+#pragma unroll
+        for (int k = 0; k < 4; ++k) {
+          const u32x4 w = *(const u32x4*)(tT + lane * TP + k * 8);
+#pragma unroll
+          for (int t = 0; t < 4; ++t) {
+            if (k * 8 + 2 * t < nvalid) sq += __uint_as_float(w[t] << 16);
+            if (k * 8 + 2 * t + 1 < nvalid) sq += __uint_as_float(w[t] & 0xFFFF0000u);
+          }
+        }
+        csum += sq;
+      }
+      unsigned short* const t_dst = g.sgd_param ? g.sgd_st1 : g.out_t;
+      const long t_ld = g.sgd_param ? g.sgd_ld1 : g.ld_t;
+      if (t_dst) {
         __builtin_amdgcn_s_waitcnt(0xc07f);
         const int part = lane & 3;
         const int mrow = m0 + wm * WTM + q * 32 + part * 8;
@@ -581,11 +610,18 @@
           const int c = ps * 16 + (lane >> 2);
           const int n = n0t + wn * WTN + c;
           if (n < g.N && mrow < g.M)
-            *(u32x4*)(g.sgd_st1 + (long)n * g.sgd_ld1 + mrow) = *(const u32x4*)(tT + c * TP + part * 8);
+            *(u32x4*)(t_dst + (long)n * t_ld + mrow) = *(const u32x4*)(tT + c * TP + part * 8);
         }
       }
     };
     quarter(IntC<0>{}); quarter(IntC<1>{}); quarter(IntC<2>{}); quarter(IntC<3>{});
+    if (g.colsum_part) {
+      float* xs = (float*)(smem + XS_OFF);
+      xs[wave * WTN + lane] = csum;
+      __syncthreads();
+      const int n = n0t + wn * WTN + lane;
+      if (wm == 0 && n < g.N) g.colsum_part[(long)bm * g.N + n] = xs[wn * WTN + lane] + xs[(NWN + wn) * WTN + lane];
+    }
   } else {
   const bool staged = g.staged_out;
   unsigned short* stile = (unsigned short*)smem + wave * (WTM * WTN);
@@ -662,12 +698,57 @@
     }
   if (staged) {
     constexpr int CPRW = WTN / 8;
+    constexpr bool SIDE = (BM == 128 && BN == 128 && WTM == 32 && WTN == 64 && sizeof(T) == 2 && AMODE == OP_KCONTIG && BMODE <= OP_KSTRIDED);
+    float cs[8];
+#pragma unroll
+    for (int t = 0; t < 8; ++t) cs[t] = 0.f;
 #pragma unroll
     for (int q = 0; q < (WTM * CPRW) / 64; ++q) {
       const int idx = q * 64 + lane, lrow = idx / CPRW, ch = idx % CPRW;
       const int m = m0 + wm * WTM + lrow, n = n0t + wn * WTN + ch * 8;
       if (m < g.M && n < g.N) {
-        __builtin_nontemporal_store(*(const u32x4*)(stile + lrow * WTN + ch * 8), (u32x4*)((unsigned short*)g.C + (long)m * g.ldc + n));
+        const u32x4 w = *(const u32x4*)(stile + lrow * WTN + ch * 8);
+        __builtin_nontemporal_store(w, (u32x4*)((unsigned short*)g.C + (long)m * g.ldc + n));
+        if (SIDE && g.colsum_part) {
+#pragma unroll
+          for (int t = 0; t < 4; ++t) { cs[2 * t] += __uint_as_float(w[t] << 16); cs[2 * t + 1] += __uint_as_float(w[t] & 0xFFFF0000u); }
+        }
+      }
+    }
+    if constexpr (SIDE) {
+      if (g.out_t) {
+        const int part = lane & 3;
+        const int mrow = m0 + wm * WTM + part * 8;
+#pragma unroll
+        for (int ps = 0; ps < WTN / 16; ++ps) {
+          const int c = ps * 16 + (lane >> 2);
+          const int n = n0t + wn * WTN + c;
+          u32x4 w;
+#pragma unroll
+          for (int t = 0; t < 4; ++t)
+            w[t] = (unsigned)stile[(part * 8 + 2 * t) * WTN + c] | ((unsigned)stile[(part * 8 + 2 * t + 1) * WTN + c] << 16);
+          if (n < g.N && mrow < g.M) *(u32x4*)(g.out_t + (long)n * g.ld_t + mrow) = w;
+        }
+      }
+      if (g.colsum_part) {
+        float* xw = (float*)stile;
+        *(f32x4*)(xw + (lane >> 3) * 64 + (lane & 7) * 8) = f32x4{cs[0], cs[1], cs[2], cs[3]};
+        *(f32x4*)(xw + (lane >> 3) * 64 + (lane & 7) * 8 + 4) = f32x4{cs[4], cs[5], cs[6], cs[7]};
+        __builtin_amdgcn_s_waitcnt(0xc07f);
+        float sw = 0.f;
+#pragma unroll
+        for (int r = 0; r < 8; ++r) sw += xw[r * 64 + lane];
+        __syncthreads();
+        float* ys = (float*)smem;
+        ys[wave * 64 + lane] = sw;
+        __syncthreads();
+        const int n = n0t + wn * WTN + lane;
+        if (wm == 0 && n < g.N) {
+          float tot = 0.f;
+#pragma unroll
+          for (int w = 0; w < BM / WTM; ++w) tot += ys[(w * NWN + wn) * 64 + lane];
+          g.colsum_part[(long)bm * g.N + n] = tot;
+        }
       }
     }
   }
@@ -958,6 +1039,18 @@
   return sgd_fused_accepts(dtype, a_kstrided, b_kstrided, M, N, K) ? 1 : 0;
 }
 
+static int side_output_parts(int dtype, int a_kstrided, int M, int N, int K) {
+  if (dtype != SW_BF16 || a_kstrided || M <= 0 || N <= 0 || (N % 8)) return 0;
+  const long t256 = (long)((M + 255) / 256) * ((N + 255) / 256);
+  if (N > 128 && t256 >= 200 && K >= 1024) return (K % 64) == 0 ? (M + 255) / 256 : 0;
+  if (N <= 64) return 0;
+  return (M + 127) / 128;
+}
+extern "C" int sw_gemm_side_output_parts(int dtype, int a_kstrided, int b_kstrided, int M, int N, int K) {
+  (void)b_kstrided;
+  return side_output_parts(dtype, a_kstrided, M, N, K);
+}
+
 extern "C" int sw_gemm(int dtype, int a_kstrided, int b_kstrided, int M, int N, int K, const void* A, long lda,
                        const void* B, long ldb, void* C, long ldc, const sw_epilogue* ep, int splitk,
                        hipStream_t stream) {
@@ -972,6 +1065,13 @@
   if (a_kstrided && (M % epc)) return -5;
   if (b_kstrided && (N % epc)) return -5;
   if (a_kstrided && !b_kstrided) return -3;
+  if (ep && (ep->colsum_part || ep->out_t)) {
+    if (!side_output_parts(dtype, a_kstrided, M, N, K) || splitk > 1 || ep->out_dtype != SW_BF16 || ep->accumulate_atomic || ep->sgd_fused || ep->fold_row_scale ||
+        (ldc % 8) || (((uintptr_t)C) & 15)) return -5;
+    if (ep->colsum_part && (((uintptr_t)ep->colsum_part) & 15)) return -4;
+    if (ep->out_t && ((M % 8) || (ep->ld_t % 8) || ep->ld_t < M)) return -5;
+    if (ep->out_t && (((uintptr_t)ep->out_t) & 15)) return -4;
+  }
   const bool plain = (!ep || (ep->out_dtype == SW_F32 && !ep->bias && !ep->relu && !ep->drop_mask && !(ep->drop_hash_p > 0.f) && !ep->relu_ref &&
                               !ep->accumulate_atomic && !ep->absmax_out && !ep->residual));
   const bool has_row_scale = ep && ep->fold_row_scale;
@@ -1054,6 +1154,7 @@
     g.ref = ep->relu_ref; g.ldr = ep->ld_ref; g.ref_scale = ep->ref_scale; g.ref_bf16 = ep->ref_dtype == SW_BF16;
     g.res = ep->residual; g.ldres = ep->ld_res; g.res_bf16 = ep->res_dtype == SW_BF16;
     g.relu = ep->relu; g.out_bf16 = ep->out_dtype == SW_BF16; g.atomic = ep->accumulate_atomic; g.absmax = ep->absmax_out;
+    g.colsum_part = ep->colsum_part; g.out_t = (unsigned short*)ep->out_t; g.ld_t = ep->ld_t;
     if (ep->sgd_fused) {
       const sw_sgd_tensor* fz = ep->sgd_fused;
       g.sgd_param = fz->param; g.sgd_mom = fz->momentum_buf; g.sgd_ld = ldc;
@@ -1129,6 +1230,7 @@
     const int rc = sw_conv3x3_direct_try(nimg, H, W, Cin, Cout, dilation, in, wk, out, ep, stream);
     if (rc != 0) return rc < 0 ? -rc : 0;
   }
+  if (ep && (ep->colsum_part || ep->out_t)) return -5;
   GemmArgs g = {};
   g.A = in; g.B = wk; g.C = out; g.M = nimg * H * W; g.N = Cout; g.K = 9 * Cin; g.lda = 0; g.ldb = 9L * Cin; g.ldc = Cout;
   g.cH = H; g.cW = W; g.cC = Cin; g.cDil = dilation;
diff --git a/sos-wsod_amd/ops.py b/sos-wsod_amd/ops.py
--- a/sos-wsod_amd/ops.py
+++ b/sos-wsod_amd/ops.py
@@ -171,6 +171,9 @@
     return torch.empty(*shape, device=dev, dtype=torch.float32)
 
 
+FUSED_SIDE_OUTPUTS = True
+
+
 def _launch(tag, fn):
     if TIMER is None or tag is None:
         return fn()
@@ -185,7 +188,7 @@
 
 def make_epilogue(bias=None, relu=False, drop_mask=None, drop_scale=2.0, relu_ref=None, ref_scale=1.0,
                   out_dtype=torch.float32, atomic=False, absmax_out=None, drop_hash=None, splitk_workspace=None, residual=None,
-                  row_scale=None):
+                  row_scale=None, colsum_part=None, out_t=None):
     ep = Epilogue()
     ep.bias = None if bias is None else bias.data_ptr()
     ep.relu = int(relu)
@@ -212,7 +215,10 @@
     ep.ld_res = 0 if residual is None else residual.stride(0)
     ep.res_dtype = SW_F32 if residual is None else dt(residual)
     ep.fold_row_scale = None if row_scale is None else row_scale.data_ptr()
-    ep._keepalive = (bias, drop_mask, relu_ref, absmax_out, splitk_workspace, drop_hash, residual, row_scale)
+    ep.colsum_part = None if colsum_part is None else colsum_part.data_ptr()
+    ep.out_t = None if out_t is None else out_t.data_ptr()
+    ep.ld_t = 0 if out_t is None else out_t.stride(0)
+    ep._keepalive = (bias, drop_mask, relu_ref, absmax_out, splitk_workspace, drop_hash, residual, row_scale, colsum_part, out_t)
     return ep
 
 
@@ -243,6 +249,10 @@
     check(_launch(tag, lambda: lib.sw_conv3x3_igemm(dt(x), n, H, W, Cin, Cout, dilation, _p(x), _p(wk), _p(out),
                                                     ctypes.byref(ep), _stream())), "sw_conv3x3_igemm")
     return out
+
+
+def conv3x3_colsum_parts(dtype, n, H, W, Cin, Cout, dilation):
+    return int(lib.sw_conv3x3_colsum_parts(dt(dtype), n, H, W, Cin, Cout, dilation))
 
 
 def conv3x3_relu_pool2(x, wk, bias, out_pooled, tag=None):
@@ -549,6 +559,10 @@
 
 def gemm_sgd_fused_supported(dtype, M, N, K, a_kstrided=False, b_kstrided=False):
     return bool(lib.sw_gemm_sgd_fused_supported(dt(dtype), int(a_kstrided), int(b_kstrided), int(M), int(N), int(K)))
+
+
+def gemm_side_output_parts(dtype, M, N, K, a_kstrided=False, b_kstrided=False):
+    return int(lib.sw_gemm_side_output_parts(dt(dtype), int(a_kstrided), int(b_kstrided), int(M), int(N), int(K)))
 
 
 def attach_sgd_fused(ep, entry, momentum, grad_scale=1.0):
diff --git a/sos-wsod_amd/roi_heads_oicrplus.py b/sos-wsod_amd/roi_heads_oicrplus.py
--- a/sos-wsod_amd/roi_heads_oicrplus.py
+++ b/sos-wsod_amd/roi_heads_oicrplus.py
@@ -498,28 +498,42 @@
         ops.gemm(dl, h2, dWh, LD, D2, M, a_kstrided=True, b_kstrided=True, splitk=4)
         dz2 = _padded(M, D2, dev, dt_)
         WhT = self._head_weights_t(Wh, dev)
-        if WhT is not None:
-            ops.gemm(dl, WhT, dz2, M, D2, LD, ep=ops.make_epilogue(relu_ref=h2, ref_scale=rs, out_dtype=dt_))
-        else:
-            ops.gemm(dl, Wh, dz2, M, D2, LD, b_kstrided=True, ep=ops.make_epilogue(relu_ref=h2, ref_scale=rs, out_dtype=dt_))
-        db2 = ops.grad_target(self.box_head.fc2.bias, (D2,), dev); ops.colsum(dz2, M, D2, db2)
         epc = 8 if dt_ == torch.bfloat16 else 4
         wgrad_nn = M % epc == 0
 
+        def side(N, K):
+            parts = ops.gemm_side_output_parts(dt_, M, N, K) if (ops.FUSED_SIDE_OUTPUTS and dt_ == torch.bfloat16 and not self.fp32x3) else 0
+            if parts == 0:
+                return {}, None, None
+            cpart = torch.empty(parts, N, device=dev, dtype=torch.float32)
+            dzt = torch.empty(N, M + 8 * epc, device=dev, dtype=dt_)[:, :M] if wgrad_nn else None
+            return dict(colsum_part=cpart, out_t=dzt), cpart, dzt
+        kw2, cpart2, dz2t = side(D2, LD)
+        if WhT is not None:
+            ops.gemm(dl, WhT, dz2, M, D2, LD, ep=ops.make_epilogue(relu_ref=h2, ref_scale=rs, out_dtype=dt_, **kw2))
+        else:
+            ops.gemm(dl, Wh, dz2, M, D2, LD, b_kstrided=True, ep=ops.make_epilogue(relu_ref=h2, ref_scale=rs, out_dtype=dt_, **kw2))
+        db2 = ops.grad_target(self.box_head.fc2.bias, (D2,), dev)
+        if cpart2 is not None:
+            ops.colsum_fold_multi([(cpart2, cpart2.shape[0], db2)])
+        else:
+            ops.colsum(dz2, M, D2, db2)
         def dz_t(dz, D):
             return ops.transpose_2d(dz, torch.empty(D, M + 8 * epc, device=dev, dtype=dt_)[:, :M], M, D)
         dW2 = ops.grad_target(self.box_head.fc2.weight, (D2, D1), dev)
         if wgrad_nn:
-            self._fc_gemm(dz_t(dz2, D2), h1, dW2, D2, D1, M, b_kstrided=True)
+            self._fc_gemm(dz2t if dz2t is not None else dz_t(dz2, D2), h1, dW2, D2, D1, M, b_kstrided=True)
         else:
             ops.gemm(dz2, h1, dW2, D2, D1, M, a_kstrided=True, b_kstrided=True)
         dz1 = _padded(M, D1, dev, dt_)
+        kw1, cpart1, dz1t = side(D1, D2)
         if st.get("W2T") is not None:
-            self._fc_gemm(dz2, st["W2T"], dz1, M, D1, D2, ep=ops.make_epilogue(relu_ref=h1, ref_scale=rs, out_dtype=dt_),
+            self._fc_gemm(dz2, st["W2T"], dz1, M, D1, D2, ep=ops.make_epilogue(relu_ref=h1, ref_scale=rs, out_dtype=dt_, **kw1),
                           wname="fc2T", wmaster=self.box_head.fc2.weight)
         else:
-            ops.gemm(dz2, W2, dz1, M, D1, D2, b_kstrided=True, ep=ops.make_epilogue(relu_ref=h1, ref_scale=rs, out_dtype=dt_))
+            ops.gemm(dz2, W2, dz1, M, D1, D2, b_kstrided=True, ep=ops.make_epilogue(relu_ref=h1, ref_scale=rs, out_dtype=dt_, **kw1))
         st["dz1"] = dz1
+        st["dz1_parts"], st["dz1_t"] = cpart1, dz1t
         dparams = [dW2, db2]
         row = 0
         for i in range(2, len(params_top), 2):
@@ -547,7 +561,9 @@
         D0, D1 = pooled.shape[1], dz1.shape[1]
 
         def nn():
-            dzt = ops.transpose_2d(dz1, torch.empty(D1, M + 64, device=dev, dtype=torch.bfloat16)[:, :M], M, D1)
+            dzt = st.get("dz1_t")
+            if dzt is None:
+                dzt = ops.transpose_2d(dz1, torch.empty(D1, M + 64, device=dev, dtype=torch.bfloat16)[:, :M], M, D1)
             scratch = torch.empty(D1, D0, device=dev, dtype=torch.float32)
             ep = ops.attach_sgd_fused(ops.make_epilogue(out_dtype=torch.float32), entry, momentum, 1.0)
             ops.gemm(dzt, pooled, scratch, D1, D0, M, b_kstrided=True, ep=ep)
@@ -560,7 +576,11 @@
         dev, M = pooled.device, st["inp"]["M"]
         D0, D1 = pooled.shape[1], dz1.shape[1]
         epc = 8 if dt_ == torch.bfloat16 else 4
-        db1 = ops.grad_target(self.box_head.fc1.bias, (D1,), dev); ops.colsum(dz1, M, D1, db1)
+        db1 = ops.grad_target(self.box_head.fc1.bias, (D1,), dev)
+        if st.get("dz1_parts") is not None:
+            ops.colsum_fold_multi([(st["dz1_parts"], st["dz1_parts"].shape[0], db1)])
+        else:
+            ops.colsum(dz1, M, D1, db1)
         plan = self._fused_fc1_plan(M, D0, D1)
         if plan is not None:
             st["fused_fc1"] = plan
@@ -571,7 +591,9 @@
         panels = getattr(self, "_fc6_panels", None)
         if panels is not None and panels[0] > 1 and D1 % (256 * panels[0]) == 0:
             rows = D1 // panels[0]
-            dzt = ops.transpose_2d(dz1, torch.empty(D1, M + 8 * epc, device=dev, dtype=dt_)[:, :M], M, D1) if M % epc == 0 else None
+            dzt = st.get("dz1_t")
+            if dzt is None and M % epc == 0:
+                dzt = ops.transpose_2d(dz1, torch.empty(D1, M + 8 * epc, device=dev, dtype=dt_)[:, :M], M, D1)
             for i in range(panels[0]):
                 if dzt is not None:
                     ops.gemm(dzt[i * rows:(i + 1) * rows], pooled, dW1[i * rows:(i + 1) * rows], rows, D0, M, b_kstrided=True)
@@ -580,7 +602,9 @@
                 panels[1](i, dW1[i * rows:(i + 1) * rows])
         elif M % epc == 0:
             def nn():
-                dzt = ops.transpose_2d(dz1, torch.empty(D1, M + 8 * epc, device=dev, dtype=dt_)[:, :M], M, D1)
+                dzt = st.get("dz1_t")
+                if dzt is None:
+                    dzt = ops.transpose_2d(dz1, torch.empty(D1, M + 8 * epc, device=dev, dtype=dt_)[:, :M], M, D1)
                 self._fc_gemm(dzt, pooled, dW1, D1, D0, M, b_kstrided=True)
             ops._launch("fc6_wgrad", nn)
         else:
```

New measurement: 501.2 images/s. No clear change (-0.3%).
